# chongminggao/CIRS-codes

Measured on AMD Instinct MI355X. Metric: simulator env-steps/s (collect + PPO update in the timed region), KuaishouEnv, higher is better.
Workload: dtype f32 (policy/tracker; rollout on the fp32 MFMA, PPO head products fp32-accurate from two fp16 pieces per operand (3 f16 MFMAs per product), fp32 accumulate) + f64 (env rewards, GAE)

## Files before the change

### cirs-codes_amd/csrc/small_gemm.h

```cpp
#pragma once
#include "common.h"

namespace cirs {

typedef float sg_f32x16 __attribute__((ext_vector_type(16)));

template <bool kNT>
__device__ __forceinline__ void rows_gemm_body(int bx, int by, const float* __restrict__ X, int ldx, const float* __restrict__ W, int ldw,
                                               const float* __restrict__ bias, int R, int Kd, int N, int relu,
                                               const float* __restrict__ relu_of, int accumulate, float* __restrict__ Y, int ldy,
                                               const long* __restrict__ out_row) {
    const int lane = threadIdx.x, hi = lane >> 5, lo = lane & 31;
    const int row0 = bx * 32, n0 = by * 32;
    const int row = row0 + lo, n = n0 + lo;
    const bool row_ok = row < R, n_ok = n < N;
    sg_f32x16 acc;
    const float b = (bias && n_ok) ? bias[n] : 0.f;
#pragma unroll
    for (int s = 0; s < 16; ++s) acc[s] = b;
    const float* xr = X + (size_t)(row_ok ? row : 0) * ldx;
    if (kNT && (Kd & 31) == 0 && (ldx & 3) == 0 && ((uintptr_t)X & 15) == 0 && (ldw & 3) == 0 && ((uintptr_t)W & 15) == 0) {
        const float* wr = W + (size_t)(n_ok ? n : 0) * ldw;
        for (int kk = 0; kk < Kd; kk += 32) {
            float a[16], bv[16];
#pragma unroll
            for (int q = 0; q < 4; ++q) {
                const float4 t = *reinterpret_cast<const float4*>(xr + kk + 16 * hi + 4 * q);
                a[4 * q] = t.x; a[4 * q + 1] = t.y; a[4 * q + 2] = t.z; a[4 * q + 3] = t.w;
            }
#pragma unroll
            for (int q = 0; q < 4; ++q) {
                const float4 t = *reinterpret_cast<const float4*>(wr + kk + 16 * hi + 4 * q);
                bv[4 * q] = t.x; bv[4 * q + 1] = t.y; bv[4 * q + 2] = t.z; bv[4 * q + 3] = t.w;
            }
#pragma unroll
            for (int j = 0; j < 16; ++j)
                acc = __builtin_amdgcn_mfma_f32_32x32x2f32(row_ok ? a[j] : 0.f, n_ok ? bv[j] : 0.f, acc, 0, 0, 0);
        }
    } else if (!kNT && (Kd & 31) == 0 && (ldx & 3) == 0 && ((uintptr_t)X & 15) == 0) {
        for (int kk = 0; kk < Kd; kk += 32) {
            float a[16], bv[16];
#pragma unroll
            for (int q = 0; q < 4; ++q) {
                const float4 t = *reinterpret_cast<const float4*>(xr + kk + 16 * hi + 4 * q);
                a[4 * q] = t.x; a[4 * q + 1] = t.y; a[4 * q + 2] = t.z; a[4 * q + 3] = t.w;
            }
#pragma unroll
            for (int j = 0; j < 16; ++j) bv[j] = n_ok ? W[(size_t)(kk + 16 * hi + j) * ldw + n] : 0.f;
#pragma unroll
            for (int j = 0; j < 16; ++j) acc = __builtin_amdgcn_mfma_f32_32x32x2f32(row_ok ? a[j] : 0.f, bv[j], acc, 0, 0, 0);
        }
    } else {
        for (int kk = 0; kk < Kd; kk += 16) {
            float a[8], bv[8];
#pragma unroll
            for (int j = 0; j < 8; ++j) {
                const int kd = kk + 2 * j + hi;
                const bool k_ok = kd < Kd;
                a[j] = (row_ok && k_ok) ? xr[kd] : 0.f;
                bv[j] = 0.f;
                if (n_ok && k_ok) bv[j] = kNT ? W[(size_t)n * ldw + kd] : W[(size_t)kd * ldw + n];
            }
#pragma unroll
            for (int j = 0; j < 8; ++j) acc = __builtin_amdgcn_mfma_f32_32x32x2f32(a[j], bv[j], acc, 0, 0, 0);
        }
    }
    if (!n_ok) return;
#pragma unroll
    for (int s = 0; s < 16; ++s) {
        const int r = row0 + (s & 3) + 8 * (s >> 2) + 4 * hi;
        if (r >= R) continue;
        const size_t o = (size_t)(out_row ? out_row[r] : (long)r) * ldy + n;
        float v = acc[s];
        if (relu) v = fmaxf(v, 0.f);
        if (relu_of && !(relu_of[o] > 0.f)) v = 0.f;
        Y[o] = accumulate ? Y[o] + v : v;
    }
}

template <bool kNT>
static __global__ __launch_bounds__(64) void rows_gemm_kernel(const float* __restrict__ X, int ldx, const float* __restrict__ W, int ldw,
                                                              const float* __restrict__ bias, int R, int Kd, int N, int relu,
                                                              const float* __restrict__ relu_of, int accumulate,
                                                              float* __restrict__ Y, int ldy,
                                                              const long* __restrict__ out_row = nullptr) {
    rows_gemm_body<kNT>(blockIdx.x, blockIdx.y, X, ldx, W, ldw, bias, R, Kd, N, relu, relu_of, accumulate, Y, ldy, out_row);
}

static inline void launch_rows_gemm(bool nt, const float* X, int ldx, const float* W, int ldw, const float* bias, int R, int Kd, int N,
                                    int relu, const float* relu_of, int accumulate, float* Y, int ldy, hipStream_t s,
                                    const long* out_row = nullptr) {
    const dim3 grid(cdiv(R, 32), cdiv(N, 32));
    if (nt) hipLaunchKernelGGL(rows_gemm_kernel<true>, grid, dim3(64), 0, s, X, ldx, W, ldw, bias, R, Kd, N, relu, relu_of, accumulate, Y, ldy, out_row);
    else hipLaunchKernelGGL(rows_gemm_kernel<false>, grid, dim3(64), 0, s, X, ldx, W, ldw, bias, R, Kd, N, relu, relu_of, accumulate, Y, ldy, out_row);
}

constexpr int kDwMaxSlabs = 256;
__host__ inline int dwg_slabs(long R) {
    const long want = (R + 63) / 64;
    return (int)(want < 1 ? 1 : (want > kDwMaxSlabs ? kDwMaxSlabs : want));
}
__host__ inline size_t dwg_partial_floats(long R, int O, int K) { return (size_t)dwg_slabs(R) * O * (K + 1); }

__device__ __forceinline__ void dw_gemm_body(int bx, int slab, const float* __restrict__ dY, int ldy, const float* __restrict__ X, int ldx, int R,
                                             int O, int K, int rows_per_slab, float* __restrict__ partial) {
    const int lane = threadIdx.x, hi = lane >> 5, lo = lane & 31;
    const int k_tiles = (K + 31) / 32;
    const int o0 = (bx / k_tiles) * 32, k0 = (bx % k_tiles) * 32;
    const int r_beg = slab * rows_per_slab, r_end = min(R, r_beg + rows_per_slab);
    const int o = o0 + lo, k = k0 + lo;
    const bool o_ok = o < O, k_ok = k < K;
    sg_f32x16 acc;
#pragma unroll
    for (int s = 0; s < 16; ++s) acc[s] = 0.f;
    float bsum = 0.f;
    for (int r = r_beg; r < r_end; r += 64) {
        float a[32], b[32];
#pragma unroll
        for (int j = 0; j < 32; ++j) {
            const int rr = r + 2 * j + hi;
            const bool r_ok = rr < r_end;
            a[j] = (r_ok && o_ok) ? dY[(size_t)rr * ldy + o] : 0.f;
            b[j] = (r_ok && k_ok) ? X[(size_t)rr * ldx + k] : 0.f;
        }
#pragma unroll
        for (int j = 0; j < 32; ++j) {
            bsum += a[j];
            acc = __builtin_amdgcn_mfma_f32_32x32x2f32(a[j], b[j], acc, 0, 0, 0);
        }
    }
    float* out = partial + (size_t)slab * O * (K + 1);
    if (k_ok) {
#pragma unroll
        for (int s = 0; s < 16; ++s) {
            const int oo = o0 + (s & 3) + 8 * (s >> 2) + 4 * hi;
            if (oo < O) out[(size_t)oo * (K + 1) + k] = acc[s];
        }
    }
    if (k0 == 0) {
        bsum += __shfl_xor(bsum, 32, CIRS_WAVE);
        if (hi == 0 && o_ok) out[(size_t)o * (K + 1) + K] = bsum;
    }
}

static __global__ __launch_bounds__(64) void dw_gemm_kernel(const float* __restrict__ dY, int ldy, const float* __restrict__ X, int ldx, int R,
                                                            int O, int K, int rows_per_slab, float* __restrict__ partial) {
    dw_gemm_body(blockIdx.x, blockIdx.y, dY, ldy, X, ldx, R, O, K, rows_per_slab, partial);
}

struct RowsGemmArgs { const float* X; int ldx; const float* W; int ldw; const float* bias; int R, Kd, N, relu; const float* relu_of; int accumulate; float* Y; int ldy; };
struct DwGemmArgs { const float* dY; int ldy; const float* X; int ldx; int R, O, K, rows_per_slab; float* partial; };
template <bool kNT>
static __global__ __launch_bounds__(64) void rows_gemm_dw_kernel(RowsGemmArgs ra, int rgx, int rgy, DwGemmArgs da, int dgx) {
    const int b = blockIdx.x;
    if (b < rgx * rgy) {
        rows_gemm_body<kNT>(b % rgx, b / rgx, ra.X, ra.ldx, ra.W, ra.ldw, ra.bias, ra.R, ra.Kd, ra.N, ra.relu, ra.relu_of, ra.accumulate, ra.Y, ra.ldy,
                            nullptr);
    } else {
        const int q = b - rgx * rgy;
        dw_gemm_body(q % dgx, q / dgx, da.dY, da.ldy, da.X, da.ldx, da.R, da.O, da.K, da.rows_per_slab, da.partial);
    }
}

static __global__ __launch_bounds__(256) void dw_gemm_final(const float* __restrict__ partial, int n_slabs, int O, int K,
                                                            float* __restrict__ dW, float* __restrict__ db) {
    const int i = blockIdx.x * blockDim.x + threadIdx.x;
    const int n_out = O * (K + 1);
    if (i >= n_out) return;
    float acc = 0.f;
    for (int c0 = 0; c0 < n_slabs; c0 += 16) {
        float t16[16];
#pragma unroll
        for (int q = 0; q < 16; ++q) t16[q] = (c0 + q < n_slabs) ? partial[(size_t)(c0 + q) * n_out + i] : 0.f;
#pragma unroll
        for (int q = 0; q < 16; ++q) acc += t16[q];
    }
    const int o = i / (K + 1), k = i % (K + 1);
    if (k < K) dW[(size_t)o * K + k] = acc;
    else if (db) db[o] = acc;
}

static inline void launch_dw_gemm(const float* dY, int ldy, const float* X, int ldx, int R, int O, int K, float* dW, float* db,
                                  float* partial, hipStream_t s) {
    const int slabs = dwg_slabs(R);
    int rows_per_slab = (R + slabs - 1) / slabs;
    rows_per_slab = (rows_per_slab + 15) & ~15;
    const int tiles = cdiv(O, 32) * cdiv(K, 32);
    hipLaunchKernelGGL(dw_gemm_kernel, dim3(tiles, slabs), dim3(64), 0, s, dY, ldy, X, ldx, R, O, K, rows_per_slab, partial);
    hipLaunchKernelGGL(dw_gemm_final, dim3(cdiv(O * (K + 1), 256)), dim3(256), 0, s, partial, slabs, O, K, dW, db);
}


struct DwJob {
    const float* dY; int ldy; const float* X; int ldx; int O; int K;
    float* dW; float* db; int tile_begin; int part_off;
};
constexpr int kMaxDwJobs = 4;
struct DwJobs { DwJob j[kMaxDwJobs]; int n; int total_tiles; int total_out; };

__device__ __forceinline__ float dw_multi_fetch(int n_out, int part_off, int n_slabs, const float* __restrict__ partial, int i) {
    float acc = 0.f;
    for (int c0 = 0; c0 < n_slabs; c0 += 32) {
        float t32[32];
#pragma unroll
        for (int q = 0; q < 32; ++q) t32[q] = (c0 + q < n_slabs) ? partial[part_off + (size_t)(c0 + q) * n_out + i] : 0.f;
#pragma unroll
        for (int q = 0; q < 32; ++q) acc += t32[q];
    }
    return acc;
}
__device__ __forceinline__ float dw_multi_fetch(const DwJob& jb, int n_slabs, const float* __restrict__ partial, int i) {
    return dw_multi_fetch(jb.O * (jb.K + 1), jb.part_off, n_slabs, partial, i);
}

static __global__ __launch_bounds__(256) void dw_multi_final(DwJobs jobs, int n_slabs, const float* __restrict__ partial) {
    int i = blockIdx.x * blockDim.x + threadIdx.x;
    if (i >= jobs.total_out) return;
    int ji = 0;
    for (; ji < jobs.n; ++ji) {
        const int n_out = jobs.j[ji].O * (jobs.j[ji].K + 1);
        if (i < n_out) break;
        i -= n_out;
    }
    const DwJob jb = jobs.j[ji];
    const int n_out = jb.O * (jb.K + 1);
    const float acc = dw_multi_fetch(jb, n_slabs, partial, i);
    const int o = i / (jb.K + 1), k = i % (jb.K + 1);
    if (k < jb.K) jb.dW[(size_t)o * jb.K + k] = acc;
    else if (jb.db) jb.db[o] = acc;
}

constexpr int kMaxDwList = 3 + 6 * CIRS_MAX_TRACKER_LAYERS;
struct DwListJob { int O, K, part_off, diag; float* dW; float* db; };
struct DwList { DwListJob j[kMaxDwList]; int n, total_out, part_floats; };

static inline void launch_rows_gemm_dw(DwList& list, const float* dwX, int dw_ldx, int dwO, int dwK, float* dW, float* db, float* partial,
                                       bool nt, const float* X, int ldx, const float* W, int ldw, const float* bias, int R, int Kd, int N,
                                       int relu, const float* relu_of, int accumulate, float* Y, int ldy, hipStream_t s) {
    const int slabs = dwg_slabs(R);
    int rows_per_slab = (R + slabs - 1) / slabs;
    rows_per_slab = (rows_per_slab + 15) & ~15;
    DwListJob& jb = list.j[list.n++];
    jb.O = dwO; jb.K = dwK; jb.part_off = list.part_floats; jb.diag = 0; jb.dW = dW; jb.db = db;
    list.part_floats += slabs * dwO * (dwK + 1);
    list.total_out += dwO * (dwK + 1);
    const int tiles = cdiv(dwO, 32) * cdiv(dwK, 32);
    const RowsGemmArgs ra{X, ldx, W, ldw, bias, R, Kd, N, relu, relu_of, accumulate, Y, ldy};
    const DwGemmArgs da{X, ldx, dwX, dw_ldx, R, dwO, dwK, rows_per_slab, partial + jb.part_off};
    const int rgx = cdiv(R, 32), rgy = cdiv(N, 32);
    if (nt) hipLaunchKernelGGL(rows_gemm_dw_kernel<true>, dim3(rgx * rgy + tiles * slabs), dim3(64), 0, s, ra, rgx, rgy, da, tiles);
    else hipLaunchKernelGGL(rows_gemm_dw_kernel<false>, dim3(rgx * rgy + tiles * slabs), dim3(64), 0, s, ra, rgx, rgy, da, tiles);
}

static __global__ __launch_bounds__(256) void dw_list_final(DwList list, int n_slabs, const float* __restrict__ partial) {
    const int g = (blockIdx.x * blockDim.x + threadIdx.x) >> 3, q = threadIdx.x & 7;
    int i = g;
    const bool live = i < list.total_out;
    if (!live) i = 0;
    int O = 1, K = 0, part_off = 0, diag = 0;
    float* dW = nullptr;
    float* db = nullptr;
    bool found = false;
#pragma unroll
    for (int ji = 0; ji < kMaxDwList; ++ji) {
        if (ji < list.n && !found) {
            const int n_out_j = list.j[ji].O * (list.j[ji].K + 1);
            if (i < n_out_j) {
                O = list.j[ji].O; K = list.j[ji].K; part_off = list.j[ji].part_off; diag = list.j[ji].diag; dW = list.j[ji].dW; db = list.j[ji].db;
                found = true;
            } else {
                i -= n_out_j;
            }
        }
    }
    const int n_out = O * (K + 1);
    const int per = (n_slabs + 7) >> 3;
    const int c_beg = q * per, c_end = min(n_slabs, c_beg + per);
    float acc = 0.f;
    for (int c0 = c_beg; c0 < c_end; c0 += 16) {
        float t16[16];
#pragma unroll
        for (int u = 0; u < 16; ++u) t16[u] = (c0 + u < c_end) ? partial[part_off + (size_t)(c0 + u) * n_out + i] : 0.f;
#pragma unroll
        for (int u = 0; u < 16; ++u) acc += t16[u];
    }
    float tot = __shfl(acc, (threadIdx.x & 63) & 56, CIRS_WAVE);
#pragma unroll
    for (int u = 1; u < 8; ++u) tot += __shfl(acc, ((threadIdx.x & 63) & 56) | u, CIRS_WAVE);
    if (!live || q != 0) return;
    const int o = i / (K + 1), k = i % (K + 1);
    if (k < K) {
        if (!diag) dW[(size_t)o * K + k] = tot;
        else if (o == k) dW[o] = tot;
    } else if (db) {
        db[o] = tot;
    }
}

static inline void launch_dw_list_final(const DwList& list, int R, const float* partial, hipStream_t s) {
    hipLaunchKernelGGL(dw_list_final, dim3(cdiv(list.total_out * 8, 256)), dim3(256), 0, s, list, dwg_slabs(R), partial);
}

__host__ inline size_t dw_list_floats(long R, int O, int K) { return (size_t)dwg_slabs(R) * O * (K + 1); }

}
```

### cirs-codes_amd/csrc/tracker_bwd.hip

```cpp
#include <algorithm>
#include "tracker_rows.h"
#include "rng.h"

namespace cirs {

#ifdef CIRS_TBWD_PROF
__device__ unsigned long long g_tbwd_prof[64];
#define CIRS_BSTAMP(K) do { if ((int)blockIdx.x == 300 && threadIdx.x == 0) g_tbwd_prof[K] = __builtin_amdgcn_s_memtime(); } while (0)
__device__ unsigned long long g_tbwd_wg[2048 * 3];
#define CIRS_BWG(SEL, WHICH) do { if ((SEL) && threadIdx.x == 0 && blockIdx.x < 2048) { g_tbwd_wg[blockIdx.x * 3 + (WHICH)] = __builtin_amdgcn_s_memtime(); \
    if ((WHICH) == 0) { unsigned hw; asm volatile("s_getreg_b32 %0, hwreg(HW_REG_HW_ID)" : "=s"(hw)); unsigned xcc; asm volatile("s_getreg_b32 %0, hwreg(HW_REG_XCC_ID)" : "=s"(xcc)); g_tbwd_wg[blockIdx.x * 3 + 2] = ((unsigned long long)xcc << 32) | hw; } } } while (0)
#else
#define CIRS_BSTAMP(K) do { } while (0)
#define CIRS_BWG(SEL, WHICH) do { } while (0)
#endif
constexpr int kChunkRows = 256;

struct DropCfg {
    int on;
    uint32_t thr;
    float inv;
    uint64_t seed;
    int env_base;
};
__device__ __forceinline__ float drop_apply(const DropCfg& dc, float v, int env, int pos, int layer, int site, int elem) {
    return dropout_keep(dc.seed, (uint32_t)(dc.env_base + env), (uint32_t)pos, (uint32_t)layer, (uint32_t)site, (uint32_t)elem, dc.thr) ? v * dc.inv : 0.f;
}
template <int NH>
__global__ __launch_bounds__(256) void attn_fwd(const float* __restrict__ QKV, const int32_t* __restrict__ row_env,
                                                const int32_t* __restrict__ row_t, const int32_t* __restrict__ offsets, int R,
                                                int Lp, float* __restrict__ P, float* __restrict__ ATT, DropCfg dc, int layer,
                                                float* __restrict__ PM) {
    extern __shared__ __attribute__((aligned(16))) float smem[];
    constexpr int HD = tD / NH;
    const int lane = threadIdx.x & 63;
    const int r = blockIdx.x * 4 + (threadIdx.x >> 6);
    if (r >= R) return;
    float* ps = smem + (size_t)(threadIdx.x >> 6) * NH * Lp;
    const int p = row_t[r], base = offsets[row_env[r]];
    const float scale = 1.0f / sqrtf((float)HD);
    float q[tD];
    {
        const f32x4* q4 = reinterpret_cast<const f32x4*>(QKV + (size_t)r * 96);
#pragma unroll
        for (int d4 = 0; d4 < tD / 4; ++d4) {
            const f32x4 t = q4[d4];
            q[4 * d4] = t.x * scale; q[4 * d4 + 1] = t.y * scale; q[4 * d4 + 2] = t.z * scale; q[4 * d4 + 3] = t.w * scale;
        }
    }
    float mx[NH], sm[NH];
#pragma unroll
    for (int h = 0; h < NH; ++h) mx[h] = -INFINITY;
    float* Pr = P + (size_t)r * NH * Lp;
    for (int jp = lane; jp <= p; jp += CIRS_WAVE) {
        float k[tD];
        {
            const f32x4* k4 = reinterpret_cast<const f32x4*>(QKV + (size_t)(base + jp) * 96 + tD);
#pragma unroll
            for (int d4 = 0; d4 < tD / 4; ++d4) {
                const f32x4 t = k4[d4];
                k[4 * d4] = t.x; k[4 * d4 + 1] = t.y; k[4 * d4 + 2] = t.z; k[4 * d4 + 3] = t.w;
            }
        }
#pragma unroll
        for (int h = 0; h < NH; ++h) {
            float sc = 0.f;
#pragma unroll
            for (int d = 0; d < HD; ++d) sc = __builtin_fmaf(q[h * HD + d], k[h * HD + d], sc);
            ps[h * Lp + jp] = sc;
            mx[h] = fmaxf(mx[h], sc);
        }
    }
#pragma unroll
    for (int h = 0; h < NH; ++h) { mx[h] = wave_max_f32(mx[h]); sm[h] = 0.f; }
    for (int jp = lane; jp <= p; jp += CIRS_WAVE) {
#pragma unroll
        for (int h = 0; h < NH; ++h) {
            const float e = expf(ps[h * Lp + jp] - mx[h]);
            ps[h * Lp + jp] = e;
            sm[h] += e;
        }
    }
#pragma unroll
    for (int h = 0; h < NH; ++h) sm[h] = 1.0f / wave_sum_f32(sm[h]);
    for (int jp = lane; jp <= p; jp += CIRS_WAVE) {
#pragma unroll
        for (int h = 0; h < NH; ++h) {
            const float pr = ps[h * Lp + jp] * sm[h];
            Pr[h * Lp + jp] = pr;
            if (dc.on) {
                const float pm = drop_apply(dc, pr, row_env[r], p, layer, CIRS_DROP_ATTN, jp * NH + h);
                PM[(size_t)r * NH * Lp + h * Lp + jp] = pm;
                ps[h * Lp + jp] = pm;
            } else {
                ps[h * Lp + jp] = pr;
            }
        }
    }
    __builtin_amdgcn_wave_barrier();
    const int half = lane >> 5, d = lane & 31, h = d / HD;
    float acc = 0.f;
    for (int j0 = half; j0 <= p; j0 += 16) {
        float v8[8];
#pragma unroll
        for (int u = 0; u < 8; ++u) v8[u] = j0 + 2 * u <= p ? QKV[(size_t)(base + j0 + 2 * u) * 96 + 2 * tD + d] : 0.f;
#pragma unroll
        for (int u = 0; u < 8; ++u)
            if (j0 + 2 * u <= p) acc = __builtin_fmaf(ps[h * Lp + j0 + 2 * u], v8[u], acc);
    }
    acc += __shfl_xor(acc, 32, CIRS_WAVE);
    if (lane < tD) ATT[(size_t)r * tD + d] = acc;
}

template <int NH>
__global__ __launch_bounds__(256) void attn_bwd_q(const float* __restrict__ QKV, const float* __restrict__ P, const float* __restrict__ dATT,
                                                  const int32_t* __restrict__ row_env, const int32_t* __restrict__ row_t,
                                                  const int32_t* __restrict__ offsets, int R, int Lp, float* __restrict__ dS,
                                                  float* __restrict__ dQKV, const float* __restrict__ PM, float drop_inv) {
    constexpr int HD = tD / NH;
    const int lane = threadIdx.x & 63;
    const int r = blockIdx.x * 4 + (threadIdx.x >> 6);
    if (r >= R) return;
    const int p = row_t[r], base = offsets[row_env[r]];
    const float scale = 1.0f / sqrtf((float)HD);
    float da[tD];
    {
        const f32x4* a4 = reinterpret_cast<const f32x4*>(dATT + (size_t)r * tD);
#pragma unroll
        for (int d4 = 0; d4 < tD / 4; ++d4) {
            const f32x4 t = a4[d4];
            da[4 * d4] = t.x; da[4 * d4 + 1] = t.y; da[4 * d4 + 2] = t.z; da[4 * d4 + 3] = t.w;
        }
    }
    const float* Pr = P + (size_t)r * NH * Lp;
    float* dSr = dS + (size_t)r * NH * Lp;
    float dot[NH];
#pragma unroll
    for (int h = 0; h < NH; ++h) dot[h] = 0.f;
    for (int jp = lane; jp <= p; jp += CIRS_WAVE) {
        float v[tD];
        {
            const f32x4* v4 = reinterpret_cast<const f32x4*>(QKV + (size_t)(base + jp) * 96 + 2 * tD);
#pragma unroll
            for (int d4 = 0; d4 < tD / 4; ++d4) {
                const f32x4 t = v4[d4];
                v[4 * d4] = t.x; v[4 * d4 + 1] = t.y; v[4 * d4 + 2] = t.z; v[4 * d4 + 3] = t.w;
            }
        }
#pragma unroll
        for (int h = 0; h < NH; ++h) {
            float dp = 0.f;
#pragma unroll
            for (int d = 0; d < HD; ++d) dp = __builtin_fmaf(da[h * HD + d], v[h * HD + d], dp);
            if (PM) dp = PM[(size_t)r * NH * Lp + h * Lp + jp] != 0.f ? dp * drop_inv : 0.f;
            dSr[h * Lp + jp] = dp;
            dot[h] = __builtin_fmaf(Pr[h * Lp + jp], dp, dot[h]);
        }
    }
#pragma unroll
    for (int h = 0; h < NH; ++h) dot[h] = wave_sum_f32(dot[h]);
    extern __shared__ float smem_q[];
    float* sds = smem_q + (size_t)(threadIdx.x >> 6) * NH * Lp;
    for (int jp = lane; jp <= p; jp += CIRS_WAVE) {
#pragma unroll
        for (int h = 0; h < NH; ++h) {
            const float ds = Pr[h * Lp + jp] * (dSr[h * Lp + jp] - dot[h]);
            dSr[h * Lp + jp] = ds;
            sds[h * Lp + jp] = ds;
        }
    }
    __builtin_amdgcn_fence(__ATOMIC_RELEASE, "wavefront");
    __builtin_amdgcn_wave_barrier();
    __builtin_amdgcn_fence(__ATOMIC_ACQUIRE, "wavefront");
    const int half = lane >> 5, d = lane & (tD - 1), hd = d / HD;
    float acc = 0.f;
    for (int j0 = half; j0 <= p; j0 += 16) {
        float k8[8];
#pragma unroll
        for (int u = 0; u < 8; ++u) k8[u] = j0 + 2 * u <= p ? QKV[(size_t)(base + j0 + 2 * u) * 96 + tD + d] : 0.f;
#pragma unroll
        for (int u = 0; u < 8; ++u)
            if (j0 + 2 * u <= p) acc = __builtin_fmaf(sds[hd * Lp + j0 + 2 * u], k8[u], acc);
    }
    acc += __shfl_xor(acc, 32, CIRS_WAVE);
    if (lane < tD) dQKV[(size_t)r * 96 + d] = acc * scale;
}

template <int NH>
__global__ __launch_bounds__(256) void attn_bwd_kv(const float* __restrict__ QKV, const float* __restrict__ P, const float* __restrict__ dS,
                                                   const float* __restrict__ dATT, const int32_t* __restrict__ row_env,
                                                   const int32_t* __restrict__ row_t, const int32_t* __restrict__ offsets,
                                                   const int32_t* __restrict__ lens, int R, int Lp, float* __restrict__ dQKV) {
    constexpr int HD = tD / NH;
    const int lane = threadIdx.x & 63;
    const int r = blockIdx.x * 4 + (threadIdx.x >> 6);
    if (r >= R) return;
    const int b = row_env[r], pk = row_t[r], base = offsets[b], len = lens[b];
    const float scale = 1.0f / sqrtf((float)HD);
    const int d = lane & (tD - 1), which = lane >> 5, h = d / HD;
    const float* coef = (which == 0 ? dS : P) + ((size_t)base * NH + h) * Lp + pk;
    const float* vec = which == 0 ? QKV + (size_t)base * 96 + d : dATT + (size_t)base * tD + d;
    const size_t cstride = (size_t)NH * Lp, vstride = which == 0 ? 96 : tD;
    const float cs = which == 0 ? scale : 1.0f;
    float acc = 0.f;
    int p = pk;
    for (; p < len; p += 8) {
        float c8[8], v8[8];
#pragma unroll
        for (int u = 0; u < 8; ++u) {
            const bool ok = p + u < len;
            c8[u] = ok ? coef[(size_t)(p + u) * cstride] : 0.f;
            v8[u] = ok ? vec[(size_t)(p + u) * vstride] : 0.f;
        }
#pragma unroll
        for (int u = 0; u < 8; ++u)
            if (p + u < len) acc = __builtin_fmaf(c8[u] * cs, v8[u], acc);
    }
    dQKV[(size_t)r * 96 + tD + lane] = acc;
}

template <int NH> struct EpGeo {
    static constexpr int NW = NH < 4 ? NH : 4;
    static constexpr int SL = 64 / NW;
    static constexpr int HPL = NH / NW;
    static constexpr int HD = tD / NH;
    static constexpr int DPL = HPL * HD;
    __host__ __device__ static constexpr int strip(int Lp) { return (HPL * Lp) | 1; }
    __host__ __device__ static constexpr size_t keep_words(int Lp) { return 2 * (size_t)NH * Lp; }
    __host__ __device__ static constexpr size_t fwd_floats(int Lp) { return (size_t)Lp * 64 + (size_t)NW * (Lp + 1) * strip(Lp) + keep_words(Lp); }
    __host__ __device__ static constexpr size_t bwd_floats(int Lp) { return (size_t)Lp * 128 + (size_t)NW * (Lp + 1) * strip(Lp) + 2 * (size_t)NH * Lp + keep_words(Lp); }
};

__device__ __forceinline__ void ep_stage(float* __restrict__ dst, const float* __restrict__ src, int rows, int src_stride, int cols, int tid, int nt) {
    const int c4n = cols >> 2;
    for (int i = tid; i < rows * c4n; i += nt) {
        const int row = i / c4n, c4 = i - row * c4n;
        *reinterpret_cast<f32x4*>(dst + (size_t)row * cols + 4 * c4) = *reinterpret_cast<const f32x4*>(src + (size_t)row * src_stride + 4 * c4);
    }
}
template <int COLS, int NQ>
__device__ __forceinline__ void ep_stage_issue(f32x4 (&r)[NQ], const float* __restrict__ src, int rows, int src_stride, int tid) {
    constexpr int c4n = COLS >> 2;
    static_assert(NQ * 64 >= 32 * c4n, "registers for 32 rows");
    const int n = rows * c4n;
#pragma unroll
    for (int q = 0; q < NQ; ++q) {
        const int i = min(tid + 64 * q, n - 1), row = i / c4n, c4 = i - row * c4n;
        r[q] = *reinterpret_cast<const f32x4*>(src + (size_t)row * src_stride + 4 * c4);
    }
}
template <int COLS, int NQ>
__device__ __forceinline__ void ep_stage_commit(float* __restrict__ dst, const f32x4 (&r)[NQ], int rows, int tid) {
    constexpr int c4n = COLS >> 2;
    const int n = rows * c4n;
#pragma unroll
    for (int q = 0; q < NQ; ++q) {
        const int i = tid + 64 * q, row = i / c4n, c4 = i - row * c4n;
        if (i < n) *reinterpret_cast<f32x4*>(dst + (size_t)row * COLS + 4 * c4) = r[q];
    }
}
__device__ __forceinline__ void ep_wave_sync() {
    asm volatile("s_waitcnt lgkmcnt(0)" ::: "memory");
    __builtin_amdgcn_wave_barrier();
}
template <int N> __device__ __forceinline__ void ep_load(float (&v)[N], const float* __restrict__ src) {
#pragma unroll
    for (int d4 = 0; d4 < N / 4; ++d4) {
        const f32x4 t = *reinterpret_cast<const f32x4*>(src + 4 * d4);
        v[4 * d4] = t.x; v[4 * d4 + 1] = t.y; v[4 * d4 + 2] = t.z; v[4 * d4 + 3] = t.w;
    }
}
template <int N> __device__ __forceinline__ void ep_store(float* __restrict__ dst, const float (&v)[N], float a) {
#pragma unroll
    for (int d4 = 0; d4 < N / 4; ++d4)
        *reinterpret_cast<f32x4*>(dst + 4 * d4) = f32x4{v[4 * d4] * a, v[4 * d4 + 1] * a, v[4 * d4 + 2] * a, v[4 * d4 + 3] * a};
}
__device__ __forceinline__ float ep_exp2(float x) { return __builtin_amdgcn_exp2f(x); }
template <int HD> __device__ __forceinline__ float ep_dot(const float* a, const float* b) {
    float s = 0.f;
#pragma unroll
    for (int d = 0; d < HD; ++d) s = __builtin_fmaf(a[d], b[d], s);
    return s;
}
template <int NH>
__device__ __forceinline__ void ep_keep_build(uint32_t* __restrict__ sK, int len, int b, int layer, const DropCfg& dc, int tid, int nt) {
    for (int i = tid; i < len * NH * 2; i += nt) sK[i] = 0u;
    ep_wave_sync();
    const int half = (len + 1) >> 1;
    const int bpr = (((len + 1) * NH + 3) >> 2) + 1;
    for (int i = tid; i < half * bpr; i += nt) {
        const int fr = i / bpr, g0 = i - fr * bpr;
        const int pA = fr, pB = len - 1 - fr;
        const int nA = ((pA + 1) * NH + 3) >> 2, nB = pB > pA ? ((pB + 1) * NH + 3) >> 2 : 0;
        const bool inA = g0 < nA;
        const int p = inA ? pA : pB, g = inA ? g0 : g0 - nA;
        if (g0 < nA + nB) {
            const u32x4 r = dropout_block(dc.seed, (uint32_t)(dc.env_base + b), (uint32_t)p, (uint32_t)layer, (uint32_t)CIRS_DROP_ATTN, (uint32_t)g);
#pragma unroll
            for (int wd = 0; wd < 4; ++wd) {
                const int elem = 4 * g + wd, j = elem / NH, h = elem - j * NH;
                if (j <= p && block_word(r, (uint32_t)wd) >= dc.thr) atomicOr(&sK[(p * NH + h) * 2 + (j >> 5)], 1u << (j & 31));
            }
        }
    }
    ep_wave_sync();
}
template <int NH>
__device__ __forceinline__ void ep_keep_build_row(uint32_t* __restrict__ sK, int p, int b, int layer, const DropCfg& dc, int tid, int nt) {
    for (int i = tid; i < NH * 2; i += nt) sK[i] = 0u;
    __syncthreads();
    for (int g = tid; 4 * g < (p + 1) * NH; g += nt) {
        const u32x4 r = dropout_block(dc.seed, (uint32_t)(dc.env_base + b), (uint32_t)p, (uint32_t)layer, (uint32_t)CIRS_DROP_ATTN, (uint32_t)g);
#pragma unroll
        for (int wd = 0; wd < 4; ++wd) {
            const int elem = 4 * g + wd, j = elem / NH, h = elem - j * NH;
            if (j <= p && block_word(r, (uint32_t)wd) >= dc.thr) atomicOr(&sK[h * 2 + (j >> 5)], 1u << (j & 31));
        }
    }
    __syncthreads();
}
__device__ __forceinline__ bool ep_keep_bit(const uint32_t (&m)[2], int j) { return ((j < 32 ? m[0] : m[1]) >> (j & 31)) & 1u; }

template <int NH, bool kDrop>
__global__ __launch_bounds__(64) void attn_fwd_ep(const float* __restrict__ QKV, const int32_t* __restrict__ offsets,
                                                  const int32_t* __restrict__ lens, int Lp, float* __restrict__ ATT, DropCfg dc, int layer,
                                                  uint32_t* __restrict__ keep_out ) {
    using G = EpGeo<NH>;
    constexpr int HPL = G::HPL, DPL = G::DPL, HD = G::HD, SL = G::SL;
    extern __shared__ __attribute__((aligned(16))) float smem[];
    const int b = blockIdx.x, len = lens[b];
    if (len <= 0) return;
    const int lane = threadIdx.x, hg = lane / SL, slot = lane - hg * SL;
    const int base = offsets[b], STR = G::strip(Lp);
    float* sKV = smem;
    float* sS = smem + (size_t)Lp * 64;
    uint32_t* sK = reinterpret_cast<uint32_t*>(sS + (size_t)G::NW * (Lp + 1) * STR);
    const int len32 = min(len, 32);
    f32x4 st_kv[8];
    ep_stage_issue<64, 8>(st_kv, QKV + (size_t)base * 96 + tD, len32, 96, lane);
    if (kDrop) {
        ep_keep_build<NH>(sK, len, b, layer, dc, lane, 64);
        if (keep_out)
            for (int i = lane; i < len * NH * 2; i += 64) keep_out[(size_t)base * NH * 2 + i] = sK[i];
    }
    ep_stage_commit<64, 8>(sKV, st_kv, len32, lane);
    if (len > 32) ep_stage(sKV + 32 * 64, QKV + (size_t)(base + 32) * 96 + tD, len - 32, 96, 64, lane, 64);
    __syncthreads();
    const float scale = 1.0f / sqrtf((float)HD), qs = scale * 1.4426950408889634f;
    for (int s0 = 0; 2 * s0 < len; s0 += SL) {
        const int pA = s0 + slot, pB = len - 1 - pA;
        const bool actA = pA <= pB, actB = pA < pB;
        const int rA = actA ? pA : 0, rB = actB ? pB : 0;
        const int jn = len - s0;
        float* myA = sS + ((size_t)hg * (Lp + 1) + (actA ? pA : Lp)) * STR;
        float* myB = sS + ((size_t)hg * (Lp + 1) + (actB ? pB : Lp)) * STR;
        float qA[DPL], qB[DPL];
        ep_load(qA, QKV + (size_t)(base + rA) * 96 + hg * DPL);
        ep_load(qB, QKV + (size_t)(base + rB) * 96 + hg * DPL);
#pragma unroll
        for (int d = 0; d < DPL; ++d) { qA[d] *= qs; qB[d] *= qs; }
        float mxA[HPL], mxB[HPL], smA[HPL], smB[HPL];
#pragma unroll
        for (int h = 0; h < HPL; ++h) { mxA[h] = mxB[h] = -INFINITY; smA[h] = smB[h] = 0.f; }
        float kq[DPL];
        ep_load(kq, sKV + hg * DPL);
#pragma unroll 4
        for (int j = 0; j < jn; ++j) {
            float k[DPL];
#pragma unroll
            for (int d = 0; d < DPL; ++d) k[d] = kq[d];
            ep_load(kq, sKV + (size_t)(j + 1 < jn ? j + 1 : j) * 64 + hg * DPL);
            const bool inA = actA && j <= pA, inB = actB && j <= pB;
#pragma unroll
            for (int h = 0; h < HPL; ++h) {
                const float sa = ep_dot<HD>(qA + h * HD, k + h * HD), sb = ep_dot<HD>(qB + h * HD, k + h * HD);
                myA[h * Lp + j] = sa; myB[h * Lp + j] = sb;
                mxA[h] = inA ? fmaxf(mxA[h], sa) : mxA[h];
                mxB[h] = inB ? fmaxf(mxB[h], sb) : mxB[h];
            }
        }
        float accA[DPL], accB[DPL];
#pragma unroll
        for (int d = 0; d < DPL; ++d) accA[d] = accB[d] = 0.f;
        uint32_t kmA[HPL][2], kmB[HPL][2];
        if (kDrop) {
#pragma unroll
            for (int h = 0; h < HPL; ++h) {
                kmA[h][0] = sK[(rA * NH + hg * HPL + h) * 2]; kmA[h][1] = sK[(rA * NH + hg * HPL + h) * 2 + 1];
                kmB[h][0] = sK[(rB * NH + hg * HPL + h) * 2]; kmB[h][1] = sK[(rB * NH + hg * HPL + h) * 2 + 1];
            }
        }
        float vq[DPL];
        ep_load(vq, sKV + 32 + hg * DPL);
#pragma unroll 4
        for (int j = 0; j < jn; ++j) {
            float v[DPL];
#pragma unroll
            for (int d = 0; d < DPL; ++d) v[d] = vq[d];
            ep_load(vq, sKV + (size_t)(j + 1 < jn ? j + 1 : j) * 64 + 32 + hg * DPL);
            const bool inA = actA && j <= pA, inB = actB && j <= pB;
#pragma unroll
            for (int h = 0; h < HPL; ++h) {
                float ea = ep_exp2(myA[h * Lp + j] - mxA[h]), eb = ep_exp2(myB[h * Lp + j] - mxB[h]);
                ea = inA ? ea : 0.f; eb = inB ? eb : 0.f;
                smA[h] += ea; smB[h] += eb;
                if (kDrop) {
                    if (!ep_keep_bit(kmA[h], j)) ea = 0.f;
                    if (!ep_keep_bit(kmB[h], j)) eb = 0.f;
                }
#pragma unroll
                for (int d = 0; d < HD; ++d) {
                    accA[h * HD + d] = __builtin_fmaf(ea, v[h * HD + d], accA[h * HD + d]);
                    accB[h * HD + d] = __builtin_fmaf(eb, v[h * HD + d], accB[h * HD + d]);
                }
            }
        }
#pragma unroll
        for (int h = 0; h < HPL; ++h) {
            const float ia = (kDrop ? dc.inv : 1.0f) / smA[h], ib = (kDrop ? dc.inv : 1.0f) / smB[h];
#pragma unroll
            for (int d = 0; d < HD; ++d) { accA[h * HD + d] *= ia; accB[h * HD + d] *= ib; }
        }
        if (actA) ep_store(ATT + (size_t)(base + pA) * tD + hg * DPL, accA, 1.0f);
        if (actB) ep_store(ATT + (size_t)(base + pB) * tD + hg * DPL, accB, 1.0f);
    }
}

template <int NH, bool kDrop>
__global__ __launch_bounds__(64) void attn_bwd_ep(const float* __restrict__ QKV, const float* __restrict__ dATT,
                                                  const int32_t* __restrict__ offsets, const int32_t* __restrict__ lens, int Lp,
                                                  float* __restrict__ dQKV, DropCfg dc, int layer,
                                                  const uint32_t* __restrict__ keep_in ) {
    using G = EpGeo<NH>;
    constexpr int HPL = G::HPL, DPL = G::DPL, HD = G::HD, SL = G::SL;
    extern __shared__ __attribute__((aligned(16))) float smem[];
    const int b = blockIdx.x, len = lens[b];
    if (len <= 0) return;
    const int lane = threadIdx.x, hg = lane / SL, slot = lane - hg * SL;
    const int base = offsets[b], STR = G::strip(Lp);
    float* sQKV = smem;
    float* sdA = smem + (size_t)Lp * 96;
    float* sS = sdA + (size_t)Lp * 32;
    float* sM = sS + (size_t)G::NW * (Lp + 1) * STR;
    float* sI = sM + (size_t)NH * Lp;
    uint32_t* sK = reinterpret_cast<uint32_t*>(sI + (size_t)NH * Lp);
    CIRS_BWG(layer == 1, 0);
    CIRS_BSTAMP(39);
    const int len32 = min(len, 32);
    f32x4 st_q[12], st_d[4];
    ep_stage_issue<96, 12>(st_q, QKV + (size_t)base * 96, len32, 96, lane);
    ep_stage_issue<tD, 4>(st_d, dATT + (size_t)base * tD, len32, tD, lane);
    CIRS_BSTAMP(38);
    if (kDrop) {
        if (keep_in) {
            for (int i = lane; i < len * NH * 2; i += 64) sK[i] = keep_in[(size_t)base * NH * 2 + i];
        } else {
            ep_keep_build<NH>(sK, len, b, layer, dc, lane, 64);
        }
    }
    ep_stage_commit<96, 12>(sQKV, st_q, len32, lane);
    ep_stage_commit<tD, 4>(sdA, st_d, len32, lane);
    if (len > 32) {
        ep_stage(sQKV + 32 * 96, QKV + (size_t)(base + 32) * 96, len - 32, 96, 96, lane, 64);
        ep_stage(sdA + 32 * tD, dATT + (size_t)(base + 32) * tD, len - 32, tD, tD, lane, 64);
    }
    __syncthreads();
    CIRS_BSTAMP(40);
    const float scale = 1.0f / sqrtf((float)HD), qs = scale * 1.4426950408889634f;
    const float dinv = kDrop ? dc.inv : 1.0f;
    for (int s0 = 0; 2 * s0 < len; s0 += SL) {
        const int pA = s0 + slot, pB = len - 1 - pA;
        const bool actA = pA <= pB, actB = pA < pB;
        const int rA = actA ? pA : 0, rB = actB ? pB : 0;
        const int jn = len - s0;
        float* myA = sS + ((size_t)hg * (Lp + 1) + (actA ? pA : Lp)) * STR;
        float* myB = sS + ((size_t)hg * (Lp + 1) + (actB ? pB : Lp)) * STR;
        float qA[DPL], qB[DPL], daA[DPL], daB[DPL];
        ep_load(qA, sQKV + (size_t)rA * 96 + hg * DPL);
        ep_load(qB, sQKV + (size_t)rB * 96 + hg * DPL);
        ep_load(daA, sdA + (size_t)rA * tD + hg * DPL);
        ep_load(daB, sdA + (size_t)rB * tD + hg * DPL);
#pragma unroll
        for (int d = 0; d < DPL; ++d) { qA[d] *= qs; qB[d] *= qs; }
        float mxA[HPL], mxB[HPL], smA[HPL], smB[HPL], dotA[HPL], dotB[HPL];
#pragma unroll
        for (int h = 0; h < HPL; ++h) { mxA[h] = mxB[h] = -INFINITY; smA[h] = smB[h] = 0.f; dotA[h] = dotB[h] = 0.f; }
        uint32_t kmA[HPL][2], kmB[HPL][2];
        if (kDrop) {
#pragma unroll
            for (int h = 0; h < HPL; ++h) {
                kmA[h][0] = sK[(rA * NH + hg * HPL + h) * 2]; kmA[h][1] = sK[(rA * NH + hg * HPL + h) * 2 + 1];
                kmB[h][0] = sK[(rB * NH + hg * HPL + h) * 2]; kmB[h][1] = sK[(rB * NH + hg * HPL + h) * 2 + 1];
            }
        }
        float kq[DPL], vq[DPL];
        ep_load(kq, sQKV + 32 + hg * DPL);
#pragma unroll 4
        for (int j = 0; j < jn; ++j) {
            float k[DPL];
#pragma unroll
            for (int d = 0; d < DPL; ++d) k[d] = kq[d];
            ep_load(kq, sQKV + (size_t)(j + 1 < jn ? j + 1 : j) * 96 + 32 + hg * DPL);
            const bool inA = actA && j <= pA, inB = actB && j <= pB;
#pragma unroll
            for (int h = 0; h < HPL; ++h) {
                const float sa = ep_dot<HD>(qA + h * HD, k + h * HD), sb = ep_dot<HD>(qB + h * HD, k + h * HD);
                myA[h * Lp + j] = sa; myB[h * Lp + j] = sb;
                mxA[h] = inA ? fmaxf(mxA[h], sa) : mxA[h];
                mxB[h] = inB ? fmaxf(mxB[h], sb) : mxB[h];
            }
        }
        CIRS_BSTAMP(45);
        ep_load(vq, sQKV + 64 + hg * DPL);
#pragma unroll 4
        for (int j = 0; j < jn; ++j) {
            float v[DPL];
#pragma unroll
            for (int d = 0; d < DPL; ++d) v[d] = vq[d];
            ep_load(vq, sQKV + (size_t)(j + 1 < jn ? j + 1 : j) * 96 + 64 + hg * DPL);
            const bool inA = actA && j <= pA, inB = actB && j <= pB;
#pragma unroll
            for (int h = 0; h < HPL; ++h) {
                float ea = ep_exp2(myA[h * Lp + j] - mxA[h]), eb = ep_exp2(myB[h * Lp + j] - mxB[h]);
                ea = inA ? ea : 0.f; eb = inB ? eb : 0.f;
                myA[h * Lp + j] = ea; myB[h * Lp + j] = eb;
                smA[h] += ea; smB[h] += eb;
                float dpa = ep_dot<HD>(daA + h * HD, v + h * HD), dpb = ep_dot<HD>(daB + h * HD, v + h * HD);
                if (kDrop) {
                    dpa = (inA && ep_keep_bit(kmA[h], j)) ? dpa * dinv : 0.f;
                    dpb = (inB && ep_keep_bit(kmB[h], j)) ? dpb * dinv : 0.f;
                }
                dotA[h] = __builtin_fmaf(ea, dpa, dotA[h]);
                dotB[h] = __builtin_fmaf(eb, dpb, dotB[h]);
            }
        }
        CIRS_BSTAMP(46);
        float invA[HPL], invB[HPL];
#pragma unroll
        for (int h = 0; h < HPL; ++h) {
            invA[h] = 1.0f / smA[h]; invB[h] = 1.0f / smB[h];
            dotA[h] *= invA[h]; dotB[h] *= invB[h];
            if (actA) { sM[((size_t)hg * Lp + pA) * HPL + h] = mxA[h]; sI[((size_t)hg * Lp + pA) * HPL + h] = invA[h]; }
            if (actB) { sM[((size_t)hg * Lp + pB) * HPL + h] = mxB[h]; sI[((size_t)hg * Lp + pB) * HPL + h] = invB[h]; }
        }
        float dqA[DPL], dqB[DPL];
#pragma unroll
        for (int d = 0; d < DPL; ++d) dqA[d] = dqB[d] = 0.f;
        ep_load(kq, sQKV + 32 + hg * DPL);
        ep_load(vq, sQKV + 64 + hg * DPL);
#pragma unroll 4
        for (int j = 0; j < jn; ++j) {
            float k[DPL], v[DPL];
#pragma unroll
            for (int d = 0; d < DPL; ++d) { k[d] = kq[d]; v[d] = vq[d]; }
            ep_load(kq, sQKV + (size_t)(j + 1 < jn ? j + 1 : j) * 96 + 32 + hg * DPL);
            ep_load(vq, sQKV + (size_t)(j + 1 < jn ? j + 1 : j) * 96 + 64 + hg * DPL);
            const bool inA = actA && j <= pA, inB = actB && j <= pB;
#pragma unroll
            for (int h = 0; h < HPL; ++h) {
                float dpa = ep_dot<HD>(daA + h * HD, v + h * HD), dpb = ep_dot<HD>(daB + h * HD, v + h * HD);
                if (kDrop) {
                    dpa = (inA && ep_keep_bit(kmA[h], j)) ? dpa * dinv : 0.f;
                    dpb = (inB && ep_keep_bit(kmB[h], j)) ? dpb * dinv : 0.f;
                }
                float dsa = myA[h * Lp + j] * invA[h] * (dpa - dotA[h]), dsb = myB[h * Lp + j] * invB[h] * (dpb - dotB[h]);
                dsa = inA ? dsa : 0.f; dsb = inB ? dsb : 0.f;
                myA[h * Lp + j] = dsa; myB[h * Lp + j] = dsb;
#pragma unroll
                for (int d = 0; d < HD; ++d) {
                    dqA[h * HD + d] = __builtin_fmaf(dsa, k[h * HD + d], dqA[h * HD + d]);
                    dqB[h * HD + d] = __builtin_fmaf(dsb, k[h * HD + d], dqB[h * HD + d]);
                }
            }
        }
        if (actA) ep_store(dQKV + (size_t)(base + pA) * 96 + hg * DPL, dqA, scale);
        if (actB) ep_store(dQKV + (size_t)(base + pB) * 96 + hg * DPL, dqB, scale);
    }
    __syncthreads();
    CIRS_BSTAMP(41);
    for (int s0 = 0; 2 * s0 < len; s0 += SL) {
        const int jA = s0 + slot, jB = len - 1 - jA;
        const bool actA = jA <= jB, actB = jA < jB;
        const int rA = actA ? jA : 0, rB = actB ? jB : 0;
        float kA[DPL], kB[DPL], dKA[DPL], dVA[DPL], dKB[DPL], dVB[DPL];
        ep_load(kA, sQKV + (size_t)rA * 96 + 32 + hg * DPL);
        ep_load(kB, sQKV + (size_t)rB * 96 + 32 + hg * DPL);
#pragma unroll
        for (int d = 0; d < DPL; ++d) { kA[d] *= qs; kB[d] *= qs; dKA[d] = dVA[d] = dKB[d] = dVB[d] = 0.f; }
        float qn[DPL], dn[DPL];
        ep_load(qn, sQKV + (size_t)s0 * 96 + hg * DPL);
        ep_load(dn, sdA + (size_t)s0 * tD + hg * DPL);
#pragma unroll 4
        for (int pq = s0; pq < len; ++pq) {
            float q[DPL], da[DPL];
#pragma unroll
            for (int d = 0; d < DPL; ++d) { q[d] = qn[d]; da[d] = dn[d]; }
            ep_load(qn, sQKV + (size_t)(pq + 1 < len ? pq + 1 : pq) * 96 + hg * DPL);
            ep_load(dn, sdA + (size_t)(pq + 1 < len ? pq + 1 : pq) * tD + hg * DPL);
            const size_t st = ((size_t)hg * Lp + pq), ss = ((size_t)hg * (Lp + 1) + pq) * STR;
            const bool inA = actA && pq >= jA, inB = actB && pq >= jB;
#pragma unroll
            for (int h = 0; h < HPL; ++h) {
                const float m = sM[st * HPL + h], iv = sI[st * HPL + h];
                float pa = ep_exp2(fminf(ep_dot<HD>(q + h * HD, kA + h * HD) - m, 0.f)) * iv;
                float pb = ep_exp2(fminf(ep_dot<HD>(q + h * HD, kB + h * HD) - m, 0.f)) * iv;
                pa = inA ? pa : 0.f; pb = inB ? pb : 0.f;
                if (kDrop) {
                    const uint32_t* kw = sK + (pq * NH + hg * HPL + h) * 2;
                    pa = (inA && ((kw[rA >> 5] >> (rA & 31)) & 1u)) ? pa * dinv : 0.f;
                    pb = (inB && ((kw[rB >> 5] >> (rB & 31)) & 1u)) ? pb * dinv : 0.f;
                }
                float dsa = sS[ss + h * Lp + rA], dsb = sS[ss + h * Lp + rB];
                dsa = inA ? dsa : 0.f; dsb = inB ? dsb : 0.f;
#pragma unroll
                for (int d = 0; d < HD; ++d) {
                    dKA[h * HD + d] = __builtin_fmaf(dsa, q[h * HD + d], dKA[h * HD + d]);
                    dVA[h * HD + d] = __builtin_fmaf(pa, da[h * HD + d], dVA[h * HD + d]);
                    dKB[h * HD + d] = __builtin_fmaf(dsb, q[h * HD + d], dKB[h * HD + d]);
                    dVB[h * HD + d] = __builtin_fmaf(pb, da[h * HD + d], dVB[h * HD + d]);
                }
            }
        }
        if (actA) {
            float* o = dQKV + (size_t)(base + jA) * 96 + 32 + hg * DPL;
            ep_store(o, dKA, scale); ep_store(o + 32, dVA, 1.0f);
        }
        if (actB) {
            float* o = dQKV + (size_t)(base + jB) * 96 + 32 + hg * DPL;
            ep_store(o, dKB, scale); ep_store(o + 32, dVB, 1.0f);
        }
    }
    CIRS_BSTAMP(42);
    CIRS_BWG(layer == 1, 1);
}
#undef EP_KEEP

constexpr int kRowT = 132;
__device__ __forceinline__ void mm_block(sg_f32x16& acc, const float (&a)[16], const float* __restrict__ wr) {
    float bv[16];
    ep_load(bv, wr);
#pragma unroll
    for (int j = 0; j < 16; ++j) acc = __builtin_amdgcn_mfma_f32_32x32x2f32(a[j], bv[j], acc, 0, 0, 0);
}
__device__ __forceinline__ void acc_to_lds(float* __restrict__ sT, const sg_f32x16& acc, int col, int hi) {
#pragma unroll
    for (int s = 0; s < 16; ++s) sT[acc_row(s, hi) * kRowT + col] = acc[s];
}
__device__ __forceinline__ void ln_half_row(const float (&y)[16], const float* __restrict__ g, const float* __restrict__ b, int hi,
                                            float (&xh)[16], float (&out)[16], float& rs) {
    float sum = 0.f;
#pragma unroll
    for (int j = 0; j < 16; ++j) sum += y[j];
    sum += __shfl_xor(sum, 32, CIRS_WAVE);
    const float mean = sum * (1.0f / tD);
    float q = 0.f;
#pragma unroll
    for (int j = 0; j < 16; ++j) { const float t = y[j] - mean; q = __builtin_fmaf(t, t, q); }
    q += __shfl_xor(q, 32, CIRS_WAVE);
    rs = 1.0f / sqrtf(q * (1.0f / tD) + 1e-5f);
    float gg[16], bb[16];
    ep_load(gg, g + 16 * hi);
    ep_load(bb, b + 16 * hi);
#pragma unroll
    for (int j = 0; j < 16; ++j) { xh[j] = (y[j] - mean) * rs; out[j] = xh[j] * gg[j] + bb[j]; }
}

struct LayerFwdArgs {
    const float *ATT, *H;
    cirs_tracker_layer y;
    const float *win_next, *bin_next;
    float *XH1, *RS1, *H1N, *FF1, *XH2, *RS2, *Hout, *QKVnext;
    const int32_t *row_env, *row_t;
    int R, layer;
};
__device__ __forceinline__ void mm_regs(sg_f32x16& acc, const float (&a)[16], const float (&bv)[16]) {
#pragma unroll
    for (int j = 0; j < 16; ++j) acc = __builtin_amdgcn_mfma_f32_32x32x2f32(a[j], bv[j], acc, 0, 0, 0);
}
__device__ __forceinline__ void ln_apply(const float (&y)[16], const float (&gg)[16], const float (&bb)[16], float (&xh)[16], float (&out)[16], float& rs) {
    float sum = 0.f;
#pragma unroll
    for (int j = 0; j < 16; ++j) sum += y[j];
    sum += __shfl_xor(sum, 32, CIRS_WAVE);
    const float mean = sum * (1.0f / tD);
    float q = 0.f;
#pragma unroll
    for (int j = 0; j < 16; ++j) { const float t = y[j] - mean; q = __builtin_fmaf(t, t, q); }
    q += __shfl_xor(q, 32, CIRS_WAVE);
    rs = 1.0f / sqrtf(q * (1.0f / tD) + 1e-5f);
#pragma unroll
    for (int j = 0; j < 16; ++j) { xh[j] = (y[j] - mean) * rs; out[j] = xh[j] * gg[j] + bb[j]; }
}
template <bool kDrop>
__global__ __launch_bounds__(64) void layer_rows_fwd(LayerFwdArgs a, DropCfg dc) {
    __shared__ __attribute__((aligned(16))) float sT[10 * 1024];
    CIRS_BSTAMP(0);
    const int lane = threadIdx.x, hi = lane >> 5, lo = lane & 31;
    const int row0 = blockIdx.x * 32, row = row0 + lo;
    const bool row_ok = row < a.R;
    const size_t rr = (size_t)(row_ok ? row : 0);
    const int env = kDrop ? a.row_env[rr] : 0, pos = kDrop ? a.row_t[rr] : 0;
    float x[16], hrow[16], wo[16], w1[4][16], g1[16], be1[16];
    ep_load(x, a.ATT + rr * tD + 16 * hi);
    ep_load(wo, a.y.out_proj_w + (size_t)lo * tD + 16 * hi);
    ep_load(hrow, a.H + rr * tD + 16 * hi);
    ep_load(g1, a.y.norm1_w + 16 * hi);
    ep_load(be1, a.y.norm1_b + 16 * hi);
#pragma unroll
    for (int nt = 0; nt < 4; ++nt) ep_load(w1[nt], a.y.lin1_w + (size_t)(nt * 32 + lo) * tD + 16 * hi);
    const float bo = a.y.out_proj_b[lo], bl2 = a.y.lin2_b[lo];
    float bl1[4];
#pragma unroll
    for (int nt = 0; nt < 4; ++nt) bl1[nt] = a.y.lin1_b[nt * 32 + lo];
    if (!row_ok) {
#pragma unroll
        for (int j = 0; j < 16; ++j) x[j] = 0.f;
    }
    sg_f32x16 acc;
#pragma unroll
    for (int s = 0; s < 16; ++s) acc[s] = bo;
    CIRS_BSTAMP(1);
    mm_regs(acc, x, wo);
    CIRS_BSTAMP(2);
    acc_to_lds(sT, acc, lo, hi);
    __syncthreads();
    float w2[4][16];
#pragma unroll
    for (int kb = 0; kb < 4; ++kb) ep_load(w2[kb], a.y.lin2_w + (size_t)lo * tH + kb * 32 + 16 * hi);
    float y[16], xh[16], h1n[16], rs;
    {
        float t[16];
        ep_load(t, sT + lo * kRowT + 16 * hi);
#pragma unroll
        for (int j = 0; j < 16; ++j) {
            float v = t[j];
            if (kDrop) v = drop_apply(dc, v, env, pos, a.layer, CIRS_DROP_RES1, 16 * hi + j);
            y[j] = row_ok ? hrow[j] + v : 0.f;
        }
    }
    CIRS_BSTAMP(3);
    ln_apply(y, g1, be1, xh, h1n, rs);
    CIRS_BSTAMP(4);
    if (row_ok) {
        ep_store(a.XH1 + rr * tD + 16 * hi, xh, 1.0f);
        ep_store(a.H1N + rr * tD + 16 * hi, h1n, 1.0f);
        if (hi == 0) a.RS1[rr] = rs;
    } else {
#pragma unroll
        for (int j = 0; j < 16; ++j) h1n[j] = 0.f;
    }
    __syncthreads();
    CIRS_BSTAMP(5);
#pragma unroll
    for (int nt = 0; nt < 4; ++nt) {
        const int n = nt * 32 + lo;
#pragma unroll
        for (int s = 0; s < 16; ++s) acc[s] = bl1[nt];
        mm_regs(acc, h1n, w1[nt]);
#pragma unroll
        for (int s = 0; s < 16; ++s) acc[s] = fmaxf(acc[s], 0.f);
        acc_to_lds(sT, acc, n, hi);
    }
    __syncthreads();
    CIRS_BSTAMP(6);
    float g2[16], be2[16], wn[3][16], bn[3];
    ep_load(g2, a.y.norm2_w + 16 * hi);
    ep_load(be2, a.y.norm2_b + 16 * hi);
    if (a.win_next) {
#pragma unroll
        for (int nt = 0; nt < 3; ++nt) {
            ep_load(wn[nt], a.win_next + (size_t)(nt * 32 + lo) * tD + 16 * hi);
            bn[nt] = a.bin_next[nt * 32 + lo];
        }
    }
#pragma unroll
    for (int s = 0; s < 16; ++s) acc[s] = bl2;
#pragma unroll
    for (int kb = 0; kb < 4; ++kb) {
        float f[16];
        ep_load(f, sT + lo * kRowT + kb * 32 + 16 * hi);
#pragma unroll
        for (int j = 0; j < 16; ++j) {
            if (kDrop) f[j] = drop_apply(dc, f[j], env, pos, a.layer, CIRS_DROP_FF, kb * 32 + 16 * hi + j);
            if (!row_ok) f[j] = 0.f;
        }
        if (row_ok) ep_store(a.FF1 + rr * tH + kb * 32 + 16 * hi, f, 1.0f);
        mm_regs(acc, f, w2[kb]);
    }
    CIRS_BSTAMP(7);
    __syncthreads();
    acc_to_lds(sT, acc, lo, hi);
    __syncthreads();
    float hn[16];
    {
        float t[16];
        ep_load(t, sT + lo * kRowT + 16 * hi);
#pragma unroll
        for (int j = 0; j < 16; ++j) {
            float v = t[j];
            if (kDrop) v = drop_apply(dc, v, env, pos, a.layer, CIRS_DROP_RES2, 16 * hi + j);
            y[j] = row_ok ? h1n[j] + v : 0.f;
        }
    }
    CIRS_BSTAMP(8);
    ln_apply(y, g2, be2, xh, hn, rs);
    CIRS_BSTAMP(9);
    if (row_ok) {
        ep_store(a.XH2 + rr * tD + 16 * hi, xh, 1.0f);
        ep_store(a.Hout + rr * tD + 16 * hi, hn, 1.0f);
        if (hi == 0) a.RS2[rr] = rs;
    } else {
#pragma unroll
        for (int j = 0; j < 16; ++j) hn[j] = 0.f;
    }
    CIRS_BSTAMP(10);
    if (a.win_next) {
#pragma unroll
        for (int nt = 0; nt < 3; ++nt) {
            const int n = nt * 32 + lo;
#pragma unroll
            for (int s = 0; s < 16; ++s) acc[s] = bn[nt];
            mm_regs(acc, hn, wn[nt]);
#pragma unroll
            for (int s = 0; s < 16; ++s) {
                const int r = row0 + acc_row(s, hi);
                if (r < a.R) a.QKVnext[(size_t)r * 96 + n] = acc[s];
            }
        }
    }
    CIRS_BSTAMP(11);
}

template <bool kDrop>
__global__ __launch_bounds__(64) void embed_inproj(const float* __restrict__ x_hist, const float* __restrict__ pe,
                                                   const int32_t* __restrict__ row_env, const int32_t* __restrict__ row_t, int R, int L,
                                                   const float* __restrict__ win, const float* __restrict__ bin, float* __restrict__ H0,
                                                   float* __restrict__ QKV, DropCfg dc) {
    const int lane = threadIdx.x, hi = lane >> 5, lo = lane & 31;
    const int row0 = blockIdx.x * 32, row = row0 + lo;
    const bool row_ok = row < R;
    const size_t rr = (size_t)(row_ok ? row : 0);
    const int b = row_env[rr], p = row_t[rr];
    float x[16], pp[16], h[16];
    ep_load(x, x_hist + ((size_t)b * L + p) * tD + 16 * hi);
    ep_load(pp, pe + (size_t)p * tD + 16 * hi);
#pragma unroll
    for (int j = 0; j < 16; ++j) {
        float v = x[j] * 5.656854249492381f + pp[j];
        if (kDrop) v = drop_apply(dc, v, b, p, 0, CIRS_DROP_POS, 16 * hi + j);
        h[j] = row_ok ? v : 0.f;
    }
    if (row_ok) ep_store(H0 + rr * tD + 16 * hi, h, 1.0f);
    sg_f32x16 acc;
#pragma unroll
    for (int nt = 0; nt < 3; ++nt) {
        const int n = nt * 32 + lo;
        const float bias = bin[n];
#pragma unroll
        for (int s = 0; s < 16; ++s) acc[s] = bias;
        mm_block(acc, h, win + (size_t)n * tD + 16 * hi);
#pragma unroll
        for (int s = 0; s < 16; ++s) {
            const int r = row0 + acc_row(s, hi);
            if (r < R) QKV[(size_t)r * 96 + n] = acc[s];
        }
    }
}

__device__ __forceinline__ void load_wcols(float (&bv)[16], const float* __restrict__ W, int ldw, int k0, int n) {
#pragma unroll
    for (int j = 0; j < 16; ++j) bv[j] = W[(size_t)(k0 + j) * ldw + n];
}
__device__ __forceinline__ void ln_bwd_half_row(const float (&dout)[16], const float (&xh)[16], const float (&gg)[16], float rs, float (&dy)[16]) {
    float s1 = 0.f, s2 = 0.f, dxh[16];
#pragma unroll
    for (int j = 0; j < 16; ++j) { dxh[j] = dout[j] * gg[j]; s1 += dxh[j]; s2 = __builtin_fmaf(dxh[j], xh[j], s2); }
    s1 += __shfl_xor(s1, 32, CIRS_WAVE);
    s2 += __shfl_xor(s2, 32, CIRS_WAVE);
    const float m1 = s1 * (1.0f / tD), m2 = s2 * (1.0f / tD);
#pragma unroll
    for (int j = 0; j < 16; ++j) dy[j] = rs * (dxh[j] - m1 - xh[j] * m2);
}
struct LayerBwdArgs {
    const float *dHin, *dY1p, *dQKVp, *winp;
    float* dHout;
    int only_pre;
    cirs_tracker_layer y;
    const float *XH2, *RS2, *FF1, *XH1, *RS1;
    float *dB2, *dFF1, *dH1N, *dY1, *dB1, *dATT;
    const int32_t *row_env, *row_t;
    int R, layer;
};
template <int LDW> __device__ __forceinline__ void load_wcols_c(float (&bv)[16], const float* __restrict__ W, int k0, int n) {
#pragma unroll
    for (int j = 0; j < 16; ++j) bv[j] = W[(k0 + j) * LDW + n];
}
template <bool kDrop>
__global__ __launch_bounds__(64) void layer_rows_bwd(LayerBwdArgs a, DropCfg dc) {
    __shared__ __attribute__((aligned(16))) float sT[10 * 1024];
    CIRS_BSTAMP(20);
    const int lane = threadIdx.x, hi = lane >> 5, lo = lane & 31;
    const int row0 = blockIdx.x * 32, row = row0 + lo;
    const bool row_ok = row < a.R;
    const size_t rr = (size_t)(row_ok ? row : 0);
    const int env = kDrop ? a.row_env[rr] : 0, pos = kDrop ? a.row_t[rr] : 0;
    const float dinv = kDrop ? dc.inv : 1.0f;
    sg_f32x16 acc;
    float dh[16];
    if (a.dQKVp) {
        float q[3][16], res[16], bv[3][16];
        ep_load(res, a.dY1p + rr * tD + 16 * hi);
#pragma unroll
        for (int kb = 0; kb < 3; ++kb) {
            ep_load(q[kb], a.dQKVp + rr * 96 + kb * 32 + 16 * hi);
            load_wcols_c<tD>(bv[kb], a.winp, kb * 32 + 16 * hi, lo);
        }
#pragma unroll
        for (int s = 0; s < 16; ++s) acc[s] = 0.f;
#pragma unroll
        for (int kb = 0; kb < 3; ++kb) {
            if (!row_ok) {
#pragma unroll
                for (int j = 0; j < 16; ++j) q[kb][j] = 0.f;
            }
            mm_regs(acc, q[kb], bv[kb]);
        }
        acc_to_lds(sT, acc, lo, hi);
        __syncthreads();
        float t[16];
        ep_load(t, sT + lo * kRowT + 16 * hi);
#pragma unroll
        for (int j = 0; j < 16; ++j) {
            dh[j] = row_ok ? res[j] + t[j] : 0.f;
            if (kDrop && a.only_pre) dh[j] = drop_apply(dc, dh[j], env, pos, 0, CIRS_DROP_POS, 16 * hi + j);
        }
        if (row_ok) ep_store(a.dHout + rr * tD + 16 * hi, dh, 1.0f);
        if (a.only_pre) return;
        __syncthreads();
    } else {
        ep_load(dh, a.dHin + rr * tD + 16 * hi);
        if (!row_ok) {
#pragma unroll
            for (int j = 0; j < 16; ++j) dh[j] = 0.f;
        }
    }
    CIRS_BSTAMP(21);
    float xh2[16], g2[16], xh1[16], g1[16], w2[4][16], ffr[4][16];
    ep_load(xh2, a.XH2 + rr * tD + 16 * hi);
    ep_load(g2, a.y.norm2_w + 16 * hi);
    const float rs2 = a.RS2[rr], rs1 = a.RS1[rr];
#pragma unroll
    for (int nt = 0; nt < 4; ++nt) load_wcols_c<tH>(w2[nt], a.y.lin2_w, 16 * hi, nt * 32 + lo);
#pragma unroll
    for (int kb = 0; kb < 4; ++kb) ep_load(ffr[kb], a.FF1 + rr * tH + kb * 32 + 16 * hi);
    ep_load(xh1, a.XH1 + rr * tD + 16 * hi);
    ep_load(g1, a.y.norm1_w + 16 * hi);
    float dy2[16], db2[16];
    ln_bwd_half_row(dh, xh2, g2, rs2, dy2);
#pragma unroll
    for (int j = 0; j < 16; ++j) {
        if (!row_ok) dy2[j] = 0.f;
        db2[j] = kDrop ? drop_apply(dc, dy2[j], env, pos, a.layer, CIRS_DROP_RES2, 16 * hi + j) : dy2[j];
    }
    if (row_ok) ep_store(a.dB2 + rr * tD + 16 * hi, db2, 1.0f);
    CIRS_BSTAMP(22);
#pragma unroll
    for (int nt = 0; nt < 4; ++nt) {
#pragma unroll
        for (int s = 0; s < 16; ++s) acc[s] = 0.f;
        mm_regs(acc, db2, w2[nt]);
        acc_to_lds(sT, acc, nt * 32 + lo, hi);
    }
    float w1[4][16], wo[16];
#pragma unroll
    for (int kb = 0; kb < 4; ++kb) load_wcols_c<tD>(w1[kb], a.y.lin1_w, kb * 32 + 16 * hi, lo);
    load_wcols_c<tD>(wo, a.y.out_proj_w, 16 * hi, lo);
    __syncthreads();
    CIRS_BSTAMP(23);
    float f[4][16];
#pragma unroll
    for (int kb = 0; kb < 4; ++kb) {
        ep_load(f[kb], sT + lo * kRowT + kb * 32 + 16 * hi);
#pragma unroll
        for (int j = 0; j < 16; ++j) f[kb][j] = (row_ok && ffr[kb][j] > 0.f) ? f[kb][j] * dinv : 0.f;
        if (row_ok) ep_store(a.dFF1 + rr * tH + kb * 32 + 16 * hi, f[kb], 1.0f);
    }
    CIRS_BSTAMP(24);
#pragma unroll
    for (int s = 0; s < 16; ++s) acc[s] = 0.f;
#pragma unroll
    for (int kb = 0; kb < 4; ++kb) mm_regs(acc, f[kb], w1[kb]);
    __syncthreads();
    acc_to_lds(sT, acc, lo, hi);
    __syncthreads();
    CIRS_BSTAMP(25);
    float dh1n[16];
    {
        float t[16];
        ep_load(t, sT + lo * kRowT + 16 * hi);
#pragma unroll
        for (int j = 0; j < 16; ++j) dh1n[j] = row_ok ? dy2[j] + t[j] : 0.f;
        if (row_ok) ep_store(a.dH1N + rr * tD + 16 * hi, dh1n, 1.0f);
    }
    CIRS_BSTAMP(26);
    float dy1[16], db1[16];
    ln_bwd_half_row(dh1n, xh1, g1, rs1, dy1);
#pragma unroll
    for (int j = 0; j < 16; ++j) {
        if (!row_ok) dy1[j] = 0.f;
        db1[j] = kDrop ? drop_apply(dc, dy1[j], env, pos, a.layer, CIRS_DROP_RES1, 16 * hi + j) : dy1[j];
    }
    if (row_ok) {
        ep_store(a.dY1 + rr * tD + 16 * hi, dy1, 1.0f);
        if (kDrop) ep_store(a.dB1 + rr * tD + 16 * hi, db1, 1.0f);
    }
    CIRS_BSTAMP(27);
#pragma unroll
    for (int s = 0; s < 16; ++s) acc[s] = 0.f;
    mm_regs(acc, db1, wo);
    __syncthreads();
    acc_to_lds(sT, acc, lo, hi);
    __syncthreads();
    {
        float t[16];
        ep_load(t, sT + lo * kRowT + 16 * hi);
        if (row_ok) ep_store(a.dATT + rr * tD + 16 * hi, t, 1.0f);
    }
    CIRS_BSTAMP(28);
}

struct BwdScratch {
    float *G, *H[CIRS_MAX_TRACKER_LAYERS + 1];
    float *QKV[CIRS_MAX_TRACKER_LAYERS], *P[CIRS_MAX_TRACKER_LAYERS], *ATT[CIRS_MAX_TRACKER_LAYERS];
    float *XH1[CIRS_MAX_TRACKER_LAYERS], *RS1[CIRS_MAX_TRACKER_LAYERS], *H1N[CIRS_MAX_TRACKER_LAYERS], *FF1[CIRS_MAX_TRACKER_LAYERS];
    float *XH2[CIRS_MAX_TRACKER_LAYERS], *RS2[CIRS_MAX_TRACKER_LAYERS];
    float *T0, *T1, *T2, *T3, *T4, *T5, *dQKV, *dFF1, *dS, *partial, *GIN;
    float* LC;
    float* PM[CIRS_MAX_TRACKER_LAYERS];
    void* sort;
};

constexpr int kLastFloats = tD + 16 + 2 + 2;

static size_t bwd_partial_floats(const cirs_tracker_cfg* cfg, long R) {
    size_t f = dw_list_floats(R, 32, tD) + dw_list_floats(R, tD, tD) + dw_list_floats(R, tD, tD + 1);
    f += (size_t)cfg->nlayers * (2 * dw_list_floats(R, tD, tD) + dw_list_floats(R, tD, tH) + dw_list_floats(R, tH, tD) +
                                 dw_list_floats(R, tD, tD) + dw_list_floats(R, 96, tD));
    return f;
}

static size_t bwd_floats(const cirs_tracker_cfg* cfg, long R) {
    const long nl = cfg->nlayers, Lp = cfg->max_len, NH = cfg->nhead;
    size_t f = 0;
    f += (size_t)R * 32;
    f += (size_t)(nl + 1) * R * tD;
    f += (size_t)nl * R * (96 + NH * Lp + tD + tD + 1 + tD + tH + tD + 1);
    f += 6 * (size_t)R * tD + (size_t)R * 96 + (size_t)R * tH + (size_t)R * NH * Lp + 64;
    if (cfg->dropout_p > 0.f) f += (size_t)nl * R * NH * Lp + 64;
    f += bwd_partial_floats(cfg, R) + 4096;
    f += (size_t)R * (tD + 1);
    f += (size_t)R * kLastFloats;
    f += emb_sort_bytes(R + cfg->n_env) / 4 + 64;
    return f + 64 * 32;
}

static BwdScratch carve_bwd(void* ws, const cirs_tracker_cfg* cfg, long R) {
    float* p = (float*)ws;
    auto take = [&](size_t n) { float* r = p; p += (n + 3) & ~(size_t)3; return r; };
    const long nl = cfg->nlayers, Lp = cfg->max_len, NH = cfg->nhead;
    BwdScratch s;
    s.G = take((size_t)R * 32);
    for (int l = 0; l <= nl; ++l) s.H[l] = take((size_t)R * tD);
    for (int l = 0; l < nl; ++l) {
        s.QKV[l] = take((size_t)R * 96); s.P[l] = take((size_t)R * NH * Lp); s.ATT[l] = take((size_t)R * tD);
        s.XH1[l] = take((size_t)R * tD); s.RS1[l] = take(R); s.H1N[l] = take((size_t)R * tD); s.FF1[l] = take((size_t)R * tH);
        s.XH2[l] = take((size_t)R * tD); s.RS2[l] = take(R);
    }
    s.T0 = take((size_t)R * tD); s.T1 = take((size_t)R * tD); s.T2 = take((size_t)R * tD); s.T3 = take((size_t)R * tD);
    s.T4 = take((size_t)R * tD); s.T5 = take((size_t)R * tD);
    for (int l = 0; l < nl; ++l) s.PM[l] = cfg->dropout_p > 0.f ? take((size_t)R * NH * Lp) : nullptr;
    s.dQKV = take((size_t)R * 96); s.dFF1 = take((size_t)R * tH); s.dS = take((size_t)R * NH * Lp);
    s.partial = take(bwd_partial_floats(cfg, R) + 4096);
    s.GIN = take((size_t)R * (tD + 1));
    s.LC = take((size_t)R * kLastFloats);
    s.sort = (void*)take(emb_sort_bytes(R + cfg->n_env) / 4 + 64);
    return s;
}

}

#ifdef CIRS_TBWD_PROF
extern "C" int cirs_debug_tbwd_wg(unsigned long long* out_host) {
    return hipMemcpyFromSymbol(out_host, HIP_SYMBOL(cirs::g_tbwd_wg), 2048 * 3 * sizeof(unsigned long long)) == hipSuccess ? 0 : -2;
}
extern "C" int cirs_debug_tbwd_prof(unsigned long long* out_host64) {
    return hipMemcpyFromSymbol(out_host64, HIP_SYMBOL(cirs::g_tbwd_prof), 64 * sizeof(unsigned long long)) == hipSuccess ? 0 : -2;
}
#endif

namespace cirs {
__global__ __launch_bounds__(256) void prefix_last_rows_kernel(const float* __restrict__ ATT, const float* __restrict__ H, const int32_t* __restrict__ row_env,
                                                               const int32_t* __restrict__ row_t, const int32_t* __restrict__ offsets,
                                                               const int32_t* __restrict__ lens, int B, float* __restrict__ ATTc, float* __restrict__ Hc,
                                                               int32_t* __restrict__ env_c, int32_t* __restrict__ t_c) {
    const int e = blockIdx.x * 8 + (threadIdx.x >> 5), c = threadIdx.x & 31;
    if (e >= B) return;
    const int n = lens[e];
    const long r = n > 0 ? (long)offsets[e] + n - 1 : -1;
    ATTc[(size_t)e * tD + c] = r >= 0 ? ATT[r * tD + c] : 0.f;
    Hc[(size_t)e * tD + c] = r >= 0 ? H[r * tD + c] : 0.f;
    if (c == 0) { env_c[e] = r >= 0 ? row_env[r] : e; t_c[e] = r >= 0 ? row_t[r] : 0; }
}
__global__ __launch_bounds__(256) void prefix_decoder_kernel(const float* __restrict__ H, const int32_t* __restrict__ lens, int B, int S,
                                                             const float* __restrict__ dec_w, const float* __restrict__ dec_b,
                                                             float* __restrict__ out, long out_stride) {
    const int e = blockIdx.x * 4 + (threadIdx.x >> 6), j = threadIdx.x & 63;
    if (e >= B || j >= S) return;
    if (lens[e] <= 0) return;
    const float* h = H + (size_t)e * tD;
    float acc = dec_b[j];
#pragma unroll
    for (int k = 0; k < tD; ++k) acc = __builtin_fmaf(h[k], dec_w[(size_t)j * tD + k], acc);
    out[(size_t)e * out_stride + j] = acc;
}

constexpr int kPQS = 104;
constexpr int kPAS = 36;
struct PrefixEnvArgs {
    const float *x_hist, *pe;
    const int32_t *row_env, *row_t, *offsets, *lens;
    cirs_tracker_layer layer[CIRS_MAX_TRACKER_LAYERS];
    const float *dec_w, *dec_b;
    float* state_out;
    long state_stride;
    int nl, L, S;
    TrunkFuse tf;
};
template <int NH> __host__ __device__ constexpr size_t prefix_env_scratch_floats() {
    return (size_t)EpGeo<NH>::NW * 33 * EpGeo<NH>::strip(32) > (size_t)32 * kRowT ? (size_t)EpGeo<NH>::NW * 33 * EpGeo<NH>::strip(32) : (size_t)32 * kRowT;
}
constexpr int kRowBitWords = 6;
template <int NH> __host__ __device__ constexpr size_t prefix_env_lds_floats() {
    return (size_t)32 * kPQS + (size_t)32 * kPAS + prefix_env_scratch_floats<NH>() + EpGeo<NH>::keep_words(32) + 32 * kRowBitWords;
}

#define EP_KEEP(POS, ELEM) dropout_keep(dc.seed, (uint32_t)(dc.env_base + b), (uint32_t)(POS), (uint32_t)layer, (uint32_t)CIRS_DROP_ATTN, (uint32_t)(ELEM), dc.thr)
template <int NH, bool kDrop>
__device__ __forceinline__ void prefix_attn_all(const float* __restrict__ sQ, float* __restrict__ sS, float* __restrict__ sA, uint32_t* __restrict__ sK, int len,
                                                int b, int layer, const DropCfg& dc, int lane) {
    using G = EpGeo<NH>;
    constexpr int HPL = G::HPL, DPL = G::DPL, HD = G::HD, SL = G::SL, Lp = 32;
    const int hg = lane / SL, slot = lane - hg * SL, STR = G::strip(Lp);
    if (kDrop) ep_keep_build<NH>(sK, len, b, layer, dc, lane, 64);
    const float scale = 1.0f / sqrtf((float)HD), qs = scale * 1.4426950408889634f;
    for (int s0 = 0; 2 * s0 < len; s0 += SL) {
        const int pA = s0 + slot, pB = len - 1 - pA;
        const bool actA = pA <= pB, actB = pA < pB;
        const int rA = actA ? pA : 0, rB = actB ? pB : 0;
        const int jn = len - s0;
        float* myA = sS + ((size_t)hg * (Lp + 1) + (actA ? pA : Lp)) * STR;
        float* myB = sS + ((size_t)hg * (Lp + 1) + (actB ? pB : Lp)) * STR;
        float qA[DPL], qB[DPL];
        ep_load(qA, sQ + rA * kPQS + hg * DPL);
        ep_load(qB, sQ + rB * kPQS + hg * DPL);
#pragma unroll
        for (int d = 0; d < DPL; ++d) { qA[d] *= qs; qB[d] *= qs; }
        float mxA[HPL], mxB[HPL], smA[HPL], smB[HPL];
#pragma unroll
        for (int h = 0; h < HPL; ++h) { mxA[h] = mxB[h] = -INFINITY; smA[h] = smB[h] = 0.f; }
        float kq[DPL];
        ep_load(kq, sQ + 32 + hg * DPL);
#pragma unroll 4
        for (int j = 0; j < jn; ++j) {
            float k[DPL];
#pragma unroll
            for (int d = 0; d < DPL; ++d) k[d] = kq[d];
            ep_load(kq, sQ + (j + 1 < jn ? j + 1 : j) * kPQS + 32 + hg * DPL);
            const bool inA = actA && j <= pA, inB = actB && j <= pB;
#pragma unroll
            for (int h = 0; h < HPL; ++h) {
                const float sa = ep_dot<HD>(qA + h * HD, k + h * HD), sb = ep_dot<HD>(qB + h * HD, k + h * HD);
                myA[h * Lp + j] = sa; myB[h * Lp + j] = sb;
                mxA[h] = inA ? fmaxf(mxA[h], sa) : mxA[h];
                mxB[h] = inB ? fmaxf(mxB[h], sb) : mxB[h];
            }
        }
        float accA[DPL], accB[DPL];
#pragma unroll
        for (int d = 0; d < DPL; ++d) accA[d] = accB[d] = 0.f;
        uint32_t kmA[HPL][2], kmB[HPL][2];
        if (kDrop) {
#pragma unroll
            for (int h = 0; h < HPL; ++h) {
                kmA[h][0] = sK[(rA * NH + hg * HPL + h) * 2]; kmA[h][1] = sK[(rA * NH + hg * HPL + h) * 2 + 1];
                kmB[h][0] = sK[(rB * NH + hg * HPL + h) * 2]; kmB[h][1] = sK[(rB * NH + hg * HPL + h) * 2 + 1];
            }
        }
        float vq[DPL];
        ep_load(vq, sQ + 64 + hg * DPL);
#pragma unroll 4
        for (int j = 0; j < jn; ++j) {
            float v[DPL];
#pragma unroll
            for (int d = 0; d < DPL; ++d) v[d] = vq[d];
            ep_load(vq, sQ + (j + 1 < jn ? j + 1 : j) * kPQS + 64 + hg * DPL);
            const bool inA = actA && j <= pA, inB = actB && j <= pB;
#pragma unroll
            for (int h = 0; h < HPL; ++h) {
                float ea = ep_exp2(myA[h * Lp + j] - mxA[h]), eb = ep_exp2(myB[h * Lp + j] - mxB[h]);
                ea = inA ? ea : 0.f; eb = inB ? eb : 0.f;
                smA[h] += ea; smB[h] += eb;
                if (kDrop) {
                    if (!ep_keep_bit(kmA[h], j)) ea = 0.f;
                    if (!ep_keep_bit(kmB[h], j)) eb = 0.f;
                }
#pragma unroll
                for (int d = 0; d < HD; ++d) {
                    accA[h * HD + d] = __builtin_fmaf(ea, v[h * HD + d], accA[h * HD + d]);
                    accB[h * HD + d] = __builtin_fmaf(eb, v[h * HD + d], accB[h * HD + d]);
                }
            }
        }
#pragma unroll
        for (int h = 0; h < HPL; ++h) {
            const float ia = (kDrop ? dc.inv : 1.0f) / smA[h], ib = (kDrop ? dc.inv : 1.0f) / smB[h];
#pragma unroll
            for (int d = 0; d < HD; ++d) { accA[h * HD + d] *= ia; accB[h * HD + d] *= ib; }
        }
        if (actA) ep_store(sA + pA * kPAS + hg * DPL, accA, 1.0f);
        if (actB) ep_store(sA + pB * kPAS + hg * DPL, accB, 1.0f);
    }
}
template <int NH, bool kDrop>
__device__ __forceinline__ void prefix_attn_last(const float* __restrict__ sQ, float* __restrict__ sS, float* __restrict__ sA, uint32_t* __restrict__ sK, int len,
                                                 int b, int layer, const DropCfg& dc, int lane) {
    constexpr int HD = tD / NH;
    const int p = len - 1;
    if (kDrop) ep_keep_build_row<NH>(sK, p, b, layer, dc, lane, 64);
    const float scale = 1.0f / sqrtf((float)HD), qs = scale * 1.4426950408889634f;
    {
        const int j = lane & 31;
        for (int h = lane >> 5; h < NH; h += 2) {
            float q[HD], k[HD];
            ep_load(q, sQ + p * kPQS + h * HD);
            ep_load(k, sQ + j * kPQS + 32 + h * HD);
#pragma unroll
            for (int d = 0; d < HD; ++d) q[d] *= qs;
            sS[h * 32 + j] = ep_dot<HD>(q, k);
        }
    }
    __syncthreads();
    if (lane < 32) {
        const int h = lane / HD;
        float sc[32];
        ep_load(sc, sS + h * 32);
        float mx = -INFINITY;
#pragma unroll
        for (int j = 0; j < 32; ++j) mx = j <= p ? fmaxf(mx, sc[j]) : mx;
        float sm = 0.f, acc = 0.f;
        const uint32_t km = kDrop ? sK[h * 2] : 0u;
#pragma unroll
        for (int j = 0; j < 32; ++j) {
            const bool in = j <= p;
            float e = ep_exp2(sc[j] - mx);
            e = in ? e : 0.f;
            sm += e;
            if (kDrop) {
                if (!((km >> j) & 1u)) e = 0.f;
            }
            acc = __builtin_fmaf(e, sQ[j * kPQS + 64 + lane], acc);
        }
        acc *= (kDrop ? dc.inv : 1.0f) / sm;
        sA[p * kPAS + lane] = acc;
    }
    __syncthreads();
}
#undef EP_KEEP
__device__ __forceinline__ void prefix_row_bits(uint32_t* __restrict__ sB, int r_begin, int n_rows, int env, int pos_of_lane, int layer, const DropCfg& dc, int lane) {
    for (int i = lane; i < 32 * kRowBitWords; i += 64) sB[i] = 0u;
    __syncthreads();
    for (int i0 = 0; i0 < n_rows * 48; i0 += 64) {
        const int i = i0 + lane, rl = i / 48, idx = i - rl * 48;
        const int pos = __shfl(pos_of_lane, (r_begin + rl) & 31, CIRS_WAVE);
        if (i < n_rows * 48) {
            const int site = idx < 8 ? (int)CIRS_DROP_RES1 : (idx < 40 ? (int)CIRS_DROP_FF : (int)CIRS_DROP_RES2);
            const int g = idx < 8 ? idx : (idx < 40 ? idx - 8 : idx - 40);
            const u32x4 r = dropout_block(dc.seed, (uint32_t)(dc.env_base + env), (uint32_t)pos, (uint32_t)layer, (uint32_t)site, (uint32_t)g);
            uint32_t m = 0u;
#pragma unroll
            for (int wd = 0; wd < 4; ++wd) m |= block_word(r, (uint32_t)wd) >= dc.thr ? 1u << wd : 0u;
            atomicOr(&sB[rl * kRowBitWords + (idx >> 3)], m << (4 * (idx & 7)));
        }
    }
    __syncthreads();
}
template <bool kDrop>
__device__ __forceinline__ void prefix_chain(const cirs_tracker_layer& y, const float* __restrict__ win_next, const float* __restrict__ bin_next, int layer,
                                             const DropCfg& dc, const uint32_t* __restrict__ myB, bool row_ok, int lo, int hi, const float* __restrict__ sA,
                                             float* __restrict__ sT, float* __restrict__ sQ, float (&hrow)[16]) {
    uint32_t kb1 = 0u, kbf[4] = {0u, 0u, 0u, 0u}, kb2 = 0u;
    if (kDrop) {
        kb1 = (myB[0] >> (16 * hi)) & 0xFFFFu;
#pragma unroll
        for (int kb = 0; kb < 4; ++kb) kbf[kb] = (myB[1 + kb] >> (16 * hi)) & 0xFFFFu;
        kb2 = (myB[5] >> (16 * hi)) & 0xFFFFu;
    }
    float x[16], wo[16], w1[4][16], g1[16], be1[16];
    ep_load(wo, y.out_proj_w + (size_t)lo * tD + 16 * hi);
    ep_load(g1, y.norm1_w + 16 * hi);
    ep_load(be1, y.norm1_b + 16 * hi);
#pragma unroll
    for (int nt = 0; nt < 4; ++nt) ep_load(w1[nt], y.lin1_w + (size_t)(nt * 32 + lo) * tD + 16 * hi);
    const float bo = y.out_proj_b[lo], bl2 = y.lin2_b[lo];
    float bl1[4];
#pragma unroll
    for (int nt = 0; nt < 4; ++nt) bl1[nt] = y.lin1_b[nt * 32 + lo];
    ep_load(x, sA + lo * kPAS + 16 * hi);
    if (!row_ok) {
#pragma unroll
        for (int j = 0; j < 16; ++j) x[j] = 0.f;
    }
    sg_f32x16 acc;
#pragma unroll
    for (int s = 0; s < 16; ++s) acc[s] = bo;
    mm_regs(acc, x, wo);
    acc_to_lds(sT, acc, lo, hi);
    __syncthreads();
    float w2[4][16];
#pragma unroll
    for (int kb = 0; kb < 4; ++kb) ep_load(w2[kb], y.lin2_w + (size_t)lo * tH + kb * 32 + 16 * hi);
    float yv[16], xh[16], h1n[16], rs;
    {
        float t[16];
        ep_load(t, sT + lo * kRowT + 16 * hi);
#pragma unroll
        for (int j = 0; j < 16; ++j) {
            float v = t[j];
            if (kDrop) v = ((kb1 >> j) & 1u) ? v * dc.inv : 0.f;
            yv[j] = row_ok ? hrow[j] + v : 0.f;
        }
    }
    ln_apply(yv, g1, be1, xh, h1n, rs);
    if (!row_ok) {
#pragma unroll
        for (int j = 0; j < 16; ++j) h1n[j] = 0.f;
    }
    __syncthreads();
#pragma unroll
    for (int nt = 0; nt < 4; ++nt) {
#pragma unroll
        for (int s = 0; s < 16; ++s) acc[s] = bl1[nt];
        mm_regs(acc, h1n, w1[nt]);
#pragma unroll
        for (int s = 0; s < 16; ++s) acc[s] = fmaxf(acc[s], 0.f);
        acc_to_lds(sT, acc, nt * 32 + lo, hi);
    }
    __syncthreads();
    float g2[16], be2[16], wn[3][16], bn[3];
    ep_load(g2, y.norm2_w + 16 * hi);
    ep_load(be2, y.norm2_b + 16 * hi);
    if (win_next) {
#pragma unroll
        for (int nt = 0; nt < 3; ++nt) {
            ep_load(wn[nt], win_next + (size_t)(nt * 32 + lo) * tD + 16 * hi);
            bn[nt] = bin_next[nt * 32 + lo];
        }
    }
#pragma unroll
    for (int s = 0; s < 16; ++s) acc[s] = bl2;
#pragma unroll
    for (int kb = 0; kb < 4; ++kb) {
        float f[16];
        ep_load(f, sT + lo * kRowT + kb * 32 + 16 * hi);
#pragma unroll
        for (int j = 0; j < 16; ++j) {
            if (kDrop) f[j] = ((kbf[kb] >> j) & 1u) ? f[j] * dc.inv : 0.f;
            if (!row_ok) f[j] = 0.f;
        }
        mm_regs(acc, f, w2[kb]);
    }
    __syncthreads();
    acc_to_lds(sT, acc, lo, hi);
    __syncthreads();
    {
        float t[16];
        ep_load(t, sT + lo * kRowT + 16 * hi);
#pragma unroll
        for (int j = 0; j < 16; ++j) {
            float v = t[j];
            if (kDrop) v = ((kb2 >> j) & 1u) ? v * dc.inv : 0.f;
            yv[j] = row_ok ? h1n[j] + v : 0.f;
        }
    }
    ln_apply(yv, g2, be2, xh, hrow, rs);
    if (!row_ok) {
#pragma unroll
        for (int j = 0; j < 16; ++j) hrow[j] = 0.f;
    }
    if (win_next) {
#pragma unroll
        for (int nt = 0; nt < 3; ++nt) {
#pragma unroll
            for (int s = 0; s < 16; ++s) acc[s] = bn[nt];
            mm_regs(acc, hrow, wn[nt]);
#pragma unroll
            for (int s = 0; s < 16; ++s) sQ[acc_row(s, hi) * kPQS + nt * 32 + lo] = acc[s];
        }
    }
    __syncthreads();
}
template <int NH, bool kDrop>
__global__ __launch_bounds__(64) void prefix_env_kernel(PrefixEnvArgs a, DropCfg dc) {
    extern __shared__ __attribute__((aligned(16))) float smem[];
    float* sQ = smem;
    float* sA = sQ + 32 * kPQS;
    float* sX = sA + 32 * kPAS;
    uint32_t* sK = reinterpret_cast<uint32_t*>(sX + prefix_env_scratch_floats<NH>());
    uint32_t* sB = sK + EpGeo<NH>::keep_words(32);
    const int e = blockIdx.x, len = a.lens[e];
    if (len <= 0) return;
    CIRS_BSTAMP(40);
    const int lane = threadIdx.x, hi = lane >> 5, lo = lane & 31;
    const int base = a.offsets[e];
    const bool row_ok = lo < len;
    const size_t rr = (size_t)base + (row_ok ? lo : 0);
    const int b = a.row_env[rr], p = a.row_t[rr];
    float h[16];
    {
        float x[16], pp[16];
        ep_load(x, a.x_hist + ((size_t)b * a.L + p) * tD + 16 * hi);
        ep_load(pp, a.pe + (size_t)p * tD + 16 * hi);
#pragma unroll
        for (int j = 0; j < 16; ++j) {
            float v = x[j] * 5.656854249492381f + pp[j];
            if (kDrop) v = drop_apply(dc, v, b, p, 0, CIRS_DROP_POS, 16 * hi + j);
            h[j] = row_ok ? v : 0.f;
        }
        sg_f32x16 acc;
        const float* win = a.layer[0].in_proj_w;
#pragma unroll
        for (int nt = 0; nt < 3; ++nt) {
            const int n = nt * 32 + lo;
            const float bias = a.layer[0].in_proj_b[n];
#pragma unroll
            for (int s = 0; s < 16; ++s) acc[s] = bias;
            mm_block(acc, h, win + (size_t)n * tD + 16 * hi);
#pragma unroll
            for (int s = 0; s < 16; ++s) sQ[acc_row(s, hi) * kPQS + n] = acc[s];
        }
    }
    __syncthreads();
    CIRS_BSTAMP(41);
    for (int l = 0; l < a.nl; ++l) {
        const bool last = l + 1 == a.nl;
        if (last) prefix_attn_last<NH, kDrop>(sQ, sX, sA, sK, len, e, l, dc, lane);
        else {
            prefix_attn_all<NH, kDrop>(sQ, sX, sA, sK, len, e, l, dc, lane);
            __syncthreads();
        }
        CIRS_BSTAMP(42 + 2 * l);
        if (kDrop) prefix_row_bits(sB, last ? len - 1 : 0, last ? 1 : len, b, p, l, dc, lane);
        prefix_chain<kDrop>(a.layer[l], last ? nullptr : a.layer[l + 1].in_proj_w, last ? nullptr : a.layer[l + 1].in_proj_b, l, dc,
                            sB + (last ? 0 : lo) * kRowBitWords, row_ok, lo, hi, sA, sX, sQ, h);
        CIRS_BSTAMP(43 + 2 * l);
    }
    if (lo == len - 1) ep_store(sA + 16 * hi, h, 1.0f);
    __syncthreads();
    float sval = 0.f;
    if (lane < a.S) {
        float acc = a.dec_b[lane];
#pragma unroll
        for (int k = 0; k < tD; ++k) acc = __builtin_fmaf(sA[k], a.dec_w[(size_t)lane * tD + k], acc);
        a.state_out[(size_t)e * a.state_stride + lane] = acc;
        sval = acc;
    }
    CIRS_BSTAMP(50);
    if (a.tf.on) {
        if (a.tf.skip && a.tf.skip[e]) {
            a.tf.h2[(size_t)e * kH + lane] = 0.f;
            if (lane == 0 && a.tf.value) a.tf.value[e] = 0.f;
            return;
        }
        float *xs = sX, *hs = sX + kH;
        if (lane < a.S) xs[lane] = sval;
        trunk_compute(a.tf.cfg, a.tf.w, xs, hs, lane, e, a.tf.h2, a.tf.value, nullptr);
    }
}

template <int NH>
__device__ __forceinline__ void last_keep_build(uint32_t* __restrict__ sK, const int32_t* __restrict__ lens, int e0, int E, int Lp, int layer,
                                                const DropCfg& dc, int tid) {
    constexpr int EPW = 64 / NH;
    for (int i = tid; i < EPW * NH * 2; i += 64) sK[i] = 0u;
    __syncthreads();
    const int gmax = (Lp * NH + 3) >> 2;
    for (int i = tid; i < EPW * gmax; i += 64) {
        const int el = i / gmax, g = i - el * gmax, e = e0 + el;
        const int len = e < E ? lens[e] : 0;
        if (4 * g < len * NH) {
            const int p = len - 1;
            const u32x4 r = dropout_block(dc.seed, (uint32_t)(dc.env_base + e), (uint32_t)p, (uint32_t)layer, (uint32_t)CIRS_DROP_ATTN, (uint32_t)g);
#pragma unroll
            for (int wd = 0; wd < 4; ++wd) {
                const int elem = 4 * g + wd, j = elem / NH, h = elem - j * NH;
                if (j <= p && block_word(r, (uint32_t)wd) >= dc.thr) atomicOr(&sK[(el * NH + h) * 2 + (j >> 5)], 1u << (j & 31));
            }
        }
    }
    __syncthreads();
}
template <int NH, bool kDrop>
__global__ __launch_bounds__(64) void attn_last_fwd(const float* __restrict__ QKV, const float* __restrict__ H, const int32_t* __restrict__ row_env,
                                                    const int32_t* __restrict__ row_t, const int32_t* __restrict__ offsets,
                                                    const int32_t* __restrict__ lens, int E, int Lp, float* __restrict__ ATTc, float* __restrict__ Hc,
                                                    float* __restrict__ stats, int32_t* __restrict__ env_c, int32_t* __restrict__ t_c, DropCfg dc, int layer) {
    constexpr int HD = tD / NH, EPW = 64 / NH;
    __shared__ uint32_t sK[EPW * NH * 2];
    const int tid = threadIdx.x, el = tid / NH, h = tid - el * NH, e0 = blockIdx.x * EPW, e = e0 + el;
    if (kDrop) last_keep_build<NH>(sK, lens, e0, E, Lp, layer, dc, tid);
    if (e >= E) return;
    const int len = lens[e];
    float acc[HD], hrow[HD];
    if (len <= 0) {
#pragma unroll
        for (int d = 0; d < HD; ++d) acc[d] = 0.f;
        ep_store(ATTc + (size_t)e * tD + h * HD, acc, 1.0f);
        ep_store(Hc + (size_t)e * tD + h * HD, acc, 1.0f);
        stats[((size_t)e * NH + h) * 2] = 0.f; stats[((size_t)e * NH + h) * 2 + 1] = 0.f;
        if (h == 0) { env_c[e] = e; t_c[e] = 0; }
        return;
    }
    const int p = len - 1;
    const size_t base = (size_t)offsets[e];
    const float* rows = QKV + base * 96 + h * HD;
    const float scale = 1.0f / sqrtf((float)HD), qs = scale * 1.4426950408889634f;
    float q[HD];
    ep_load(q, rows + (size_t)p * 96);
    ep_load(hrow, H + (base + p) * tD + h * HD);
#pragma unroll
    for (int d = 0; d < HD; ++d) q[d] *= qs;
    float mx = -INFINITY;
#pragma unroll 4
    for (int j = 0; j <= p; ++j) {
        float k[HD];
        ep_load(k, rows + (size_t)j * 96 + 32);
        mx = fmaxf(mx, ep_dot<HD>(q, k));
    }
    uint32_t km[2] = {0u, 0u};
    if (kDrop) { km[0] = sK[(el * NH + h) * 2]; km[1] = sK[(el * NH + h) * 2 + 1]; }
    float sm = 0.f;
#pragma unroll
    for (int d = 0; d < HD; ++d) acc[d] = 0.f;
#pragma unroll 4
    for (int j = 0; j <= p; ++j) {
        float k[HD], v[HD];
        ep_load(k, rows + (size_t)j * 96 + 32);
        ep_load(v, rows + (size_t)j * 96 + 64);
        float ex = ep_exp2(ep_dot<HD>(q, k) - mx);
        sm += ex;
        if (kDrop) {
            if (!ep_keep_bit(km, j)) ex = 0.f;
        }
#pragma unroll
        for (int d = 0; d < HD; ++d) acc[d] = __builtin_fmaf(ex, v[d], acc[d]);
    }
    const float ia = (kDrop ? dc.inv : 1.0f) / sm;
#pragma unroll
    for (int d = 0; d < HD; ++d) acc[d] *= ia;
    ep_store(ATTc + (size_t)e * tD + h * HD, acc, 1.0f);
    ep_store(Hc + (size_t)e * tD + h * HD, hrow, 1.0f);
    stats[((size_t)e * NH + h) * 2] = mx; stats[((size_t)e * NH + h) * 2 + 1] = 1.0f / sm;
    if (h == 0) { env_c[e] = row_env[base + p]; t_c[e] = row_t[base + p]; }
}
template <int NH, bool kDrop>
__global__ __launch_bounds__(64) void attn_last_bwd(const float* __restrict__ QKV, const float* __restrict__ dATTc, const float* __restrict__ dY1c,
                                                    const float* __restrict__ stats, const int32_t* __restrict__ offsets, const int32_t* __restrict__ lens,
                                                    int E, int Lp, float* __restrict__ dQKV, float* __restrict__ dY1, DropCfg dc, int layer) {
    constexpr int HD = tD / NH, EPW = 64 / NH;
    __shared__ uint32_t sK[EPW * NH * 2];
    const int tid = threadIdx.x, el = tid / NH, h = tid - el * NH, e0 = blockIdx.x * EPW, e = e0 + el;
    if (kDrop) last_keep_build<NH>(sK, lens, e0, E, Lp, layer, dc, tid);
    if (e >= E) return;
    const int len = lens[e];
    if (len <= 0) return;
    const int p = len - 1;
    const size_t base = (size_t)offsets[e];
    const float* rows = QKV + base * 96 + h * HD;
    const float scale = 1.0f / sqrtf((float)HD), qs = scale * 1.4426950408889634f, dinv = kDrop ? dc.inv : 1.0f;
    float qr[HD], q[HD], da[HD], res[HD], zero[HD];
    ep_load(qr, rows + (size_t)p * 96);
    ep_load(da, dATTc + (size_t)e * tD + h * HD);
    ep_load(res, dY1c + (size_t)e * tD + h * HD);
#pragma unroll
    for (int d = 0; d < HD; ++d) { q[d] = qr[d] * qs; zero[d] = 0.f; }
    const float mx = stats[((size_t)e * NH + h) * 2], inv = stats[((size_t)e * NH + h) * 2 + 1];
    uint32_t km[2] = {0u, 0u};
    if (kDrop) { km[0] = sK[(el * NH + h) * 2]; km[1] = sK[(el * NH + h) * 2 + 1]; }
    float dot = 0.f;
#pragma unroll 4
    for (int j = 0; j <= p; ++j) {
        float k[HD], v[HD];
        ep_load(k, rows + (size_t)j * 96 + 32);
        ep_load(v, rows + (size_t)j * 96 + 64);
        const float ex = ep_exp2(ep_dot<HD>(q, k) - mx);
        float dp = ep_dot<HD>(da, v);
        if (kDrop) dp = ep_keep_bit(km, j) ? dp * dinv : 0.f;
        dot = __builtin_fmaf(ex, dp, dot);
    }
    dot *= inv;
    float dq[HD];
#pragma unroll
    for (int d = 0; d < HD; ++d) dq[d] = 0.f;
    float* orow = dQKV + base * 96 + h * HD;
    float* yrow = dY1 + base * tD + h * HD;
#pragma unroll 2
    for (int j = 0; j <= p; ++j) {
        float k[HD], v[HD];
        ep_load(k, rows + (size_t)j * 96 + 32);
        ep_load(v, rows + (size_t)j * 96 + 64);
        const float pj = ep_exp2(ep_dot<HD>(q, k) - mx) * inv;
        float dp = ep_dot<HD>(da, v), pm = pj;
        if (kDrop) {
            const bool keep = ep_keep_bit(km, j);
            dp = keep ? dp * dinv : 0.f;
            pm = keep ? pj * dinv : 0.f;
        }
        const float ds = pj * (dp - dot);
#pragma unroll
        for (int d = 0; d < HD; ++d) dq[d] = __builtin_fmaf(ds, k[d], dq[d]);
        ep_store(orow + (size_t)j * 96 + 32, qr, ds * scale);
        ep_store(orow + (size_t)j * 96 + 64, da, pm);
        if (j < p) {
            ep_store(orow + (size_t)j * 96, zero, 1.0f);
            ep_store(yrow + (size_t)j * tD, zero, 1.0f);
        }
    }
    ep_store(orow + (size_t)p * 96, dq, scale);
    ep_store(yrow + (size_t)p * tD, res, 1.0f);
}
__global__ __launch_bounds__(256) void dstate_last_rows(const float* __restrict__ dstate_last, const int32_t* __restrict__ lens, int E, int S,
                                                        float* __restrict__ G) {
    const long i = blockIdx.x * (long)blockDim.x + threadIdx.x;
    if (i >= (long)E * S) return;
    G[i] = lens[i / S] > 0 ? dstate_last[i] : 0.f;
}
__global__ __launch_bounds__(256) void dstate_last_full(const float* __restrict__ dstate_last, const int32_t* __restrict__ row_env,
                                                        const int32_t* __restrict__ offsets, const int32_t* __restrict__ lens, int R, int S,
                                                        float* __restrict__ G) {
    const long i = blockIdx.x * (long)blockDim.x + threadIdx.x;
    if (i >= (long)R * S) return;
    const int r = (int)(i / S), s = (int)(i % S), b = row_env[r];
    G[i] = r == offsets[b] + lens[b] - 1 ? dstate_last[(size_t)b * S + s] : 0.f;
}
}

extern "C" int64_t cirs_tracker_backward_workspace_bytes(const cirs_tracker_cfg* cfg, int32_t n_rows) {
    if (!cfg || n_rows <= 0) return 0;
    return (int64_t)cirs::bwd_floats(cfg, n_rows) * 4;
}

static inline size_t spread_dyn_lds(long n_blocks, size_t static_bytes, size_t dyn_bytes) {
    if (n_blocks > cirs::device_cu_count()) return dyn_bytes;
    const size_t want = 81 * 1024;
    return static_bytes + dyn_bytes >= want ? dyn_bytes : want - static_bytes;
}
template <typename K> static inline void lds_optin(K k, size_t dyn) {
    if (dyn > 8 * 1024) (void)hipFuncSetAttribute(reinterpret_cast<const void*>(k), hipFuncAttributeMaxDynamicSharedMemorySize, (int)dyn);
}
#define CIRS_LAUNCH_SPREAD(KERNEL, GRID, STATIC_B, DYN_B, STREAM, ...)                                  \
    do {                                                                                               \
        const size_t dyn_ = spread_dyn_lds((long)(GRID), (STATIC_B), (DYN_B));                         \
        if (dyn_ != (size_t)(DYN_B)) lds_optin(KERNEL, dyn_);                                          \
        hipLaunchKernelGGL(KERNEL, dim3(GRID), dim3(64), dyn_, STREAM, __VA_ARGS__);                   \
    } while (0)

static int tracker_rows_impl(const cirs_tracker_cfg* cfg, const cirs_tracker_weights* w, const cirs_tracker_state* st,
                             const int32_t* users, const int64_t* act, const double* rew, const int32_t* row_env,
                             const int32_t* row_t, const int32_t* offsets, const int32_t* lens, int32_t n_rows,
                             const float* dstate, const cirs_tracker_grads* grads, void* workspace,
                             int64_t workspace_bytes, void* stream, float* state_out, int64_t state_stride, const float* dstate_last = nullptr,
                             const cirs::TrunkFuse* ptf = nullptr, int* ptf_fused = nullptr) {
    using namespace cirs;
    CIRS_REQUIRE(cfg && w && st && row_env && row_t && offsets && lens && workspace, "null argument");
    CIRS_REQUIRE(state_out || (users && act && rew && (dstate || dstate_last) && grads), "null argument");
    if (cfg->dim_model != tD || cfg->d_hid != tH) return fail(CIRS_E_UNSUPPORTED, "dim_model == 32 and d_hid == 128 only");
    CIRS_REQUIRE(cfg->nhead == 1 || cfg->nhead == 2 || cfg->nhead == 4 || cfg->nhead == 8, "nhead must be 1,2,4,8");
    CIRS_REQUIRE(n_rows > 0, "n_rows must be positive");
    const int n_carve = dstate_last && cfg->n_env > n_rows ? cfg->n_env : n_rows;
    CIRS_REQUIRE(workspace_bytes >= cirs_tracker_backward_workspace_bytes(cfg, n_carve), "workspace too small");
    hipStream_t s = (hipStream_t)stream;
    const int R = n_rows, B = cfg->n_env, S = cfg->dim_state, L = cfg->max_len, NH = cfg->nhead, nl = cfg->nlayers;
    BwdScratch sc = carve_bwd(workspace, cfg, n_carve);
    auto g1 = [&](long n) { return dim3(cdiv(n, 256)); };

    DwList dwl{};
#define ATT_DISPATCH_SH(KERNEL, SHMEM, ...)                                                               \
    do {                                                                                                  \
        switch (NH) {                                                                                     \
            case 1: hipLaunchKernelGGL(KERNEL<1>, dim3(cdiv(R, 4)), dim3(256), SHMEM, s, __VA_ARGS__); break; \
            case 2: hipLaunchKernelGGL(KERNEL<2>, dim3(cdiv(R, 4)), dim3(256), SHMEM, s, __VA_ARGS__); break; \
            case 4: hipLaunchKernelGGL(KERNEL<4>, dim3(cdiv(R, 4)), dim3(256), SHMEM, s, __VA_ARGS__); break; \
            default: hipLaunchKernelGGL(KERNEL<8>, dim3(cdiv(R, 4)), dim3(256), SHMEM, s, __VA_ARGS__); break; \
        }                                                                                                 \
    } while (0)
#define ATT_DISPATCH(KERNEL, ...) ATT_DISPATCH_SH(KERNEL, 0, __VA_ARGS__)
    auto ep_bytes = [&](bool bwd) -> size_t {
        switch (NH) {
            case 1: return 4 * (bwd ? EpGeo<1>::bwd_floats(L) : EpGeo<1>::fwd_floats(L));
            case 2: return 4 * (bwd ? EpGeo<2>::bwd_floats(L) : EpGeo<2>::fwd_floats(L));
            case 4: return 4 * (bwd ? EpGeo<4>::bwd_floats(L) : EpGeo<4>::fwd_floats(L));
            default: return 4 * (bwd ? EpGeo<8>::bwd_floats(L) : EpGeo<8>::fwd_floats(L));
        }
    };
    const bool ep = L <= 64 && ep_bytes(true) <= 64 * 1024 && !getenv("CIRS_TRACKER_ATTN_ROWS");
#define ATT_EP1(KERNEL, N, BWD, ...)                                                                                            \
    do {                                                                                                                        \
        if (dc.on) CIRS_LAUNCH_SPREAD((KERNEL<N, true>), B, 0, ep_bytes(BWD), s, __VA_ARGS__);       \
        else CIRS_LAUNCH_SPREAD((KERNEL<N, false>), B, 0, ep_bytes(BWD), s, __VA_ARGS__);           \
    } while (0)
#define ATT_EP(KERNEL, BWD, ...)                                  \
    do {                                                          \
        switch (NH) {                                             \
            case 1: ATT_EP1(KERNEL, 1, BWD, __VA_ARGS__); break;  \
            case 2: ATT_EP1(KERNEL, 2, BWD, __VA_ARGS__); break;  \
            case 4: ATT_EP1(KERNEL, 4, BWD, __VA_ARGS__); break;  \
            default: ATT_EP1(KERNEL, 8, BWD, __VA_ARGS__); break; \
        }                                                         \
    } while (0)

    DropCfg dc{};
    if (cfg->dropout_p > 0.f) {
        CIRS_REQUIRE(cfg->dropout_p < 1.f, "dropout_p must be in [0, 1)");
        dc.on = 1; dc.thr = dropout_threshold(cfg->dropout_p); dc.inv = 1.0f / (1.0f - cfg->dropout_p);
        dc.seed = cfg->dropout_seed; dc.env_base = cfg->drop_env_base;
    }
    if (state_out && ep && L <= 32 && S <= 64 && !getenv("CIRS_TRACKER_PREFIX_LAUNCHES")) {
        PrefixEnvArgs pa{};
        pa.x_hist = st->x_hist; pa.pe = w->pe; pa.row_env = row_env; pa.row_t = row_t; pa.offsets = offsets; pa.lens = lens;
        for (int l = 0; l < nl; ++l) pa.layer[l] = w->layer[l];
        pa.dec_w = w->dec_w; pa.dec_b = w->dec_b; pa.state_out = state_out; pa.state_stride = (long)state_stride; pa.nl = nl; pa.L = L; pa.S = S;
        if (ptf && ptf->on) {
            CIRS_REQUIRE(ptf->cfg.hidden == kH && ptf->cfg.dim_state == S && ptf->h2, "prefix states: trunk shape mismatch");
            pa.tf = *ptf;
            if (ptf_fused) *ptf_fused = 1;
        }
#define PREFIX_ENV(N)                                                                                                                        \
    do {                                                                                                                                     \
        const size_t sh = std::max<size_t>(4 * prefix_env_lds_floats<N>(), 40 * 1024);           \
        if (dc.on) hipLaunchKernelGGL((prefix_env_kernel<N, true>), dim3(B), dim3(64), sh, s, pa, dc);                                        \
        else hipLaunchKernelGGL((prefix_env_kernel<N, false>), dim3(B), dim3(64), sh, s, pa, dc);                                             \
    } while (0)
        switch (NH) {
            case 1: PREFIX_ENV(1); break;
            case 2: PREFIX_ENV(2); break;
            case 4: PREFIX_ENV(4); break;
            default: PREFIX_ENV(8); break;
        }
#undef PREFIX_ENV
        CIRS_CHECK_LAUNCH("prefix_env_kernel");
        return CIRS_OK;
    }
    if (dc.on) CIRS_LAUNCH_SPREAD(embed_inproj<true>, cdiv(R, 32), 0, 0, s, st->x_hist, w->pe, row_env, row_t, R, L, w->layer[0].in_proj_w,
                                  w->layer[0].in_proj_b, sc.H[0], sc.QKV[0], dc);
    else CIRS_LAUNCH_SPREAD(embed_inproj<false>, cdiv(R, 32), 0, 0, s, st->x_hist, w->pe, row_env, row_t, R, L, w->layer[0].in_proj_w,
                            w->layer[0].in_proj_b, sc.H[0], sc.QKV[0], dc);
    const bool top_last = dstate_last && ep && nl >= 2 && !getenv("CIRS_TRACKER_LAST_FULL");
    float *dY1c = sc.LC, *att_stats = sc.LC + (size_t)B * tD;
    int32_t *env_c = reinterpret_cast<int32_t*>(att_stats + (size_t)B * 16), *t_c = env_c + B;
#define ATT_LAST1(KERNEL, N, ...)                                                                                        \
    do {                                                                                                                 \
        if (dc.on) hipLaunchKernelGGL((KERNEL<N, true>), dim3(cdiv(B, 64 / N)), dim3(64), 0, s, __VA_ARGS__);             \
        else hipLaunchKernelGGL((KERNEL<N, false>), dim3(cdiv(B, 64 / N)), dim3(64), 0, s, __VA_ARGS__);                  \
    } while (0)
#define ATT_LAST(KERNEL, ...)                                  \
    do {                                                       \
        switch (NH) {                                          \
            case 1: ATT_LAST1(KERNEL, 1, __VA_ARGS__); break;  \
            case 2: ATT_LAST1(KERNEL, 2, __VA_ARGS__); break;  \
            case 4: ATT_LAST1(KERNEL, 4, __VA_ARGS__); break;  \
            default: ATT_LAST1(KERNEL, 8, __VA_ARGS__); break; \
        }                                                      \
    } while (0)
    for (int l = 0; l < nl; ++l) {
        const cirs_tracker_layer& y = w->layer[l];
        if (top_last && l == nl - 1) {
            float* Hc = sc.T1;
            ATT_LAST(attn_last_fwd, (const float*)sc.QKV[l], (const float*)sc.H[l], row_env, row_t, offsets, lens, B, L, sc.ATT[l], Hc, att_stats, env_c, t_c,
                     dc, l);
            LayerFwdArgs fa{sc.ATT[l], Hc, y, nullptr, nullptr, sc.XH1[l], sc.RS1[l], sc.H1N[l], sc.FF1[l], sc.XH2[l], sc.RS2[l], sc.H[l + 1], nullptr,
                            env_c, t_c, B, l};
            if (dc.on) CIRS_LAUNCH_SPREAD(layer_rows_fwd<true>, cdiv(B, 32), 40 * 1024, 0, s, fa, dc);
            else CIRS_LAUNCH_SPREAD(layer_rows_fwd<false>, cdiv(B, 32), 40 * 1024, 0, s, fa, dc);
            continue;
        }
        if (ep) ATT_EP(attn_fwd_ep, false, (const float*)sc.QKV[l], offsets, lens, L, sc.ATT[l], dc, l, (dc.on && !state_out) ? reinterpret_cast<uint32_t*>(sc.P[l]) : (uint32_t*)nullptr);
        else ATT_DISPATCH_SH(attn_fwd, (size_t)4 * NH * L * sizeof(float), sc.QKV[l], row_env, row_t, offsets, R, L, sc.P[l], sc.ATT[l], dc, l, sc.PM[l]);
        if (state_out && l == nl - 1) {
            static_assert(tD == 32, "prefix_last_rows_kernel maps 32 columns to 32 threads");
            float *ATTc = sc.T0, *Hc = sc.T1;
            int32_t *env_c = reinterpret_cast<int32_t*>(sc.T2), *t_c = env_c + B;
            hipLaunchKernelGGL(prefix_last_rows_kernel, dim3(cdiv(B, 8)), dim3(256), 0, s, (const float*)sc.ATT[l], (const float*)sc.H[l], row_env, row_t, offsets,
                               lens, B, ATTc, Hc, env_c, t_c);
            LayerFwdArgs fa{ATTc, Hc, y, nullptr, nullptr, sc.XH1[l], sc.RS1[l], sc.H1N[l], sc.FF1[l], sc.XH2[l], sc.RS2[l], sc.H[l + 1], nullptr,
                            env_c, t_c, B, l};
            if (dc.on) CIRS_LAUNCH_SPREAD(layer_rows_fwd<true>, cdiv(B, 32), 40 * 1024, 0, s, fa, dc);
            else CIRS_LAUNCH_SPREAD(layer_rows_fwd<false>, cdiv(B, 32), 40 * 1024, 0, s, fa, dc);
            continue;
        }
        LayerFwdArgs fa{sc.ATT[l], sc.H[l], y, l + 1 < nl ? w->layer[l + 1].in_proj_w : nullptr, l + 1 < nl ? w->layer[l + 1].in_proj_b : nullptr,
                        sc.XH1[l], sc.RS1[l], sc.H1N[l], sc.FF1[l], sc.XH2[l], sc.RS2[l], sc.H[l + 1], l + 1 < nl ? sc.QKV[l + 1] : nullptr,
                        row_env, row_t, R, l};
        if (dc.on) CIRS_LAUNCH_SPREAD(layer_rows_fwd<true>, cdiv(R, 32), 40 * 1024, 0, s, fa, dc);
        else CIRS_LAUNCH_SPREAD(layer_rows_fwd<false>, cdiv(R, 32), 40 * 1024, 0, s, fa, dc);
    }
    CIRS_CHECK_LAUNCH("tracker forward recompute");
    if (state_out) {
        hipLaunchKernelGGL(prefix_decoder_kernel, dim3(cdiv(B, 4)), dim3(256), 0, s, (const float*)sc.H[nl], lens, B, S, w->dec_w, w->dec_b,
                           state_out, (long)state_stride);
        CIRS_CHECK_LAUNCH("prefix_decoder_kernel");
        return CIRS_OK;
    }
    float* dH = sc.T0;
    if (top_last) {
        hipLaunchKernelGGL(dstate_last_rows, g1((long)B * S), dim3(256), 0, s, dstate_last, lens, B, S, sc.G);
        launch_rows_gemm(false, sc.G, S, w->dec_w, tD, nullptr, B, S, tD, 0, nullptr, 0, dH, tD, s);
    } else {
        if (dstate_last) hipLaunchKernelGGL(dstate_last_full, g1((long)R * S), dim3(256), 0, s, dstate_last, row_env, offsets, lens, R, S, sc.G);
        else hipLaunchKernelGGL(gather_dstate, g1((long)R * S), dim3(256), 0, s, dstate, row_env, row_t, R, S, B, sc.G);
        launch_rows_gemm_dw(dwl, sc.H[nl], tD, S, tD, grads->dec_w, grads->dec_b, sc.partial, false, sc.G, S, w->dec_w, tD, nullptr, R, S, tD, 0, nullptr, 0,
                            dH, tD, s);
    }
    for (int l = nl - 1; l >= 0; --l) {
        const cirs_tracker_layer& y = w->layer[l];
        const cirs_tracker_layer_grads& gy = grads->layer[l];
        if (top_last && l == nl - 1) {
            float* dB1 = dc.on ? sc.T4 : dY1c;
            LayerBwdArgs ba{sc.T0, nullptr, nullptr, nullptr, sc.T0, 0, y, sc.XH2[l], sc.RS2[l], sc.FF1[l], sc.XH1[l], sc.RS1[l], sc.T3, sc.dFF1, sc.T1, dY1c, dB1,
                            sc.T5, env_c, t_c, B, l};
            if (dc.on) CIRS_LAUNCH_SPREAD(layer_rows_bwd<true>, cdiv(B, 32), 40 * 1024, 0, s, ba, dc);
            else CIRS_LAUNCH_SPREAD(layer_rows_bwd<false>, cdiv(B, 32), 40 * 1024, 0, s, ba, dc);
            DwBatch bt{};
            dw_batch_add(bt, dwl, sc.G, S, sc.H[nl], tD, R, S, tD, grads->dec_w, grads->dec_b, 0, sc.partial);
            dw_batch_add(bt, dwl, sc.T0, tD, sc.XH2[l], tD, R, tD, tD, gy.norm2_w, gy.norm2_b, 1, sc.partial);
            dw_batch_add(bt, dwl, sc.T3, tD, sc.FF1[l], tH, R, tD, tH, gy.lin2_w, gy.lin2_b, 0, sc.partial);
            dw_batch_add(bt, dwl, sc.dFF1, tH, sc.H1N[l], tD, R, tH, tD, gy.lin1_w, gy.lin1_b, 0, sc.partial);
            dw_batch_add(bt, dwl, sc.T1, tD, sc.XH1[l], tD, R, tD, tD, gy.norm1_w, gy.norm1_b, 1, sc.partial);
            dw_batch_add(bt, dwl, dB1, tD, sc.ATT[l], tD, R, tD, tD, gy.out_proj_w, gy.out_proj_b, 0, sc.partial);
            dw_batch_launch(bt, R, s, B);
            ATT_LAST(attn_last_bwd, (const float*)sc.QKV[l], (const float*)sc.T5, (const float*)dY1c, (const float*)att_stats, offsets, lens, B, L, sc.dQKV,
                     sc.T2, dc, l);
            continue;
        }
        const bool pre = l + 1 < nl;
        float* dB1 = dc.on ? sc.T4 : sc.T2;
        LayerBwdArgs ba{sc.T0, pre ? sc.T2 : nullptr, pre ? sc.dQKV : nullptr, pre ? w->layer[l + 1].in_proj_w : nullptr, sc.T0, 0, y,
                        sc.XH2[l], sc.RS2[l], sc.FF1[l], sc.XH1[l], sc.RS1[l], sc.T3, sc.dFF1, sc.T1, sc.T2, dB1, sc.T5, row_env, row_t, R, l};
        if (dc.on) CIRS_LAUNCH_SPREAD(layer_rows_bwd<true>, cdiv(R, 32), 40 * 1024, 0, s, ba, dc);
        else CIRS_LAUNCH_SPREAD(layer_rows_bwd<false>, cdiv(R, 32), 40 * 1024, 0, s, ba, dc);
        DwBatch bt{};
        if (pre) dw_batch_add(bt, dwl, sc.dQKV, 96, sc.H[l + 1], tD, R, 96, tD, grads->layer[l + 1].in_proj_w, grads->layer[l + 1].in_proj_b, 0, sc.partial);
        dw_batch_add(bt, dwl, sc.T0, tD, sc.XH2[l], tD, R, tD, tD, gy.norm2_w, gy.norm2_b, 1, sc.partial);
        dw_batch_add(bt, dwl, sc.T3, tD, sc.FF1[l], tH, R, tD, tH, gy.lin2_w, gy.lin2_b, 0, sc.partial);
        dw_batch_add(bt, dwl, sc.dFF1, tH, sc.H1N[l], tD, R, tH, tD, gy.lin1_w, gy.lin1_b, 0, sc.partial);
        dw_batch_add(bt, dwl, sc.T1, tD, sc.XH1[l], tD, R, tD, tD, gy.norm1_w, gy.norm1_b, 1, sc.partial);
        dw_batch_add(bt, dwl, dB1, tD, sc.ATT[l], tD, R, tD, tD, gy.out_proj_w, gy.out_proj_b, 0, sc.partial);
        dw_batch_launch(bt, R, s);
        const float* dATT = sc.T5;
        if (ep) {
            ATT_EP(attn_bwd_ep, true, (const float*)sc.QKV[l], dATT, offsets, lens, L, sc.dQKV, dc, l, dc.on ? reinterpret_cast<const uint32_t*>(sc.P[l]) : (const uint32_t*)nullptr);
        } else {
            ATT_DISPATCH_SH(attn_bwd_q, (size_t)4 * NH * L * sizeof(float), sc.QKV[l], sc.P[l], dATT, row_env, row_t, offsets, R, L, sc.dS, sc.dQKV,
                            (const float*)sc.PM[l], dc.inv);
            ATT_DISPATCH(attn_bwd_kv, sc.QKV[l], dc.on ? sc.PM[l] : sc.P[l], sc.dS, dATT, row_env, row_t, offsets, lens, R, L, sc.dQKV);
        }
    }
    {
        LayerBwdArgs ba{};
        ba.dY1p = sc.T2; ba.dQKVp = sc.dQKV; ba.winp = w->layer[0].in_proj_w; ba.dHout = sc.T0; ba.only_pre = 1;
        ba.row_env = row_env; ba.row_t = row_t; ba.R = R;
        if (dc.on) CIRS_LAUNCH_SPREAD(layer_rows_bwd<true>, cdiv(R, 32), 40 * 1024, 0, s, ba, dc);
        else CIRS_LAUNCH_SPREAD(layer_rows_bwd<false>, cdiv(R, 32), 40 * 1024, 0, s, ba, dc);
    }
    CIRS_CHECK_LAUNCH("tracker backward layers");
    float* DU = sc.T1;
    float* EU = sc.H[nl];
    float* DPRE = sc.H1N[0];
    float* CU = sc.QKV[0];
    float* CI = sc.QKV[0] + (size_t)R * tD;
    int32_t* key_user = (int32_t*)sc.RS1[0];
    int32_t* key_item = (int32_t*)sc.RS2[0];
    const bool merged = B <= R;
    const int slot_rpw = R >= (1 << 17) ? 8 : 1;
    hipLaunchKernelGGL(slot_bwd, dim3(cdiv(R, 4 * slot_rpw)), dim3(256), 0, s, *w, dH, users, act, rew, row_env, row_t, R, B, DU, EU, DPRE,
                       sc.GIN, CU, CI, key_user, key_item, merged ? CI + (size_t)R * tD : nullptr, slot_rpw, 5.656854249492381f);
    if (merged) {
        if (int rc = emb_scatter_merged(key_item, users, lens, CI, R, B, cfg->n_items, cfg->n_users, grads->emb_item, grads->emb_user, sc.sort,
                                        emb_sort_bytes(R + B), s)) return rc;
    } else {
        int32_t* keys_c = (int32_t*)sc.T0;
        float* contrib_c = sc.T2;
        CIRS_HIP(hipMemsetAsync(keys_c, 0xFF, sizeof(int32_t) * (size_t)B, s));
        hipLaunchKernelGGL(compact_user_rows, dim3(cdiv(R, 8)), dim3(256), 0, s, row_env, row_t, users, (const float*)CU, R, keys_c, contrib_c);
        if (int rc = emb_scatter_sorted(keys_c, contrib_c, B, cfg->n_users, grads->emb_user, sc.sort, emb_sort_bytes(R), s)) return rc;
        if (int rc = emb_scatter_sorted(key_item, CI, R, cfg->n_items, grads->emb_item, sc.sort, emb_sort_bytes(R), s)) return rc;
    }
    DwBatch bt{};
    dw_batch_add(bt, dwl, sc.dQKV, 96, sc.H[0], tD, R, 96, tD, grads->layer[0].in_proj_w, grads->layer[0].in_proj_b, 0, sc.partial);
    dw_batch_add(bt, dwl, DU, tD, EU, tD, R, tD, tD, grads->ffn_user_w, grads->ffn_user_b, 0, sc.partial);
    dw_batch_add(bt, dwl, DPRE, tD, sc.GIN, tD + 1, R, tD, tD + 1, grads->gate_w, grads->gate_b, 0, sc.partial);
    dw_batch_launch(bt, R, s);
    launch_dw_list_final(dwl, R, sc.partial, s);
    CIRS_CHECK_LAUNCH("tracker backward slots");
#undef ATT_LAST
#undef ATT_LAST1
#undef ATT_DISPATCH
#undef ATT_EP
#undef ATT_EP1
#undef ATT_DISPATCH_SH
    return CIRS_OK;
}

extern "C" int cirs_tracker_backward(const cirs_tracker_cfg* cfg, const cirs_tracker_weights* w, const cirs_tracker_state* st,
                                     const int32_t* users, const int64_t* act, const double* rew, const int32_t* row_env,
                                     const int32_t* row_t, const int32_t* offsets, const int32_t* lens, int32_t n_rows,
                                     const float* dstate, const cirs_tracker_grads* grads, void* workspace,
                                     int64_t workspace_bytes, void* stream) {
    CIRS_REQUIRE(users && act && rew && dstate && grads, "null argument");
    return tracker_rows_impl(cfg, w, st, users, act, rew, row_env, row_t, offsets, lens, n_rows, dstate, grads, workspace, workspace_bytes, stream,
                             nullptr, 0);
}

extern "C" int cirs_tracker_backward_last(const cirs_tracker_cfg* cfg, const cirs_tracker_weights* w, const cirs_tracker_state* st,
                                          const int32_t* users, const int64_t* act, const double* rew, const int32_t* row_env,
                                          const int32_t* row_t, const int32_t* offsets, const int32_t* lens, int32_t n_rows,
                                          const float* dstate_last, const cirs_tracker_grads* grads, void* workspace,
                                          int64_t workspace_bytes, void* stream) {
    CIRS_REQUIRE(users && act && rew && dstate_last && grads, "null argument");
    return tracker_rows_impl(cfg, w, st, users, act, rew, row_env, row_t, offsets, lens, n_rows, nullptr, grads, workspace, workspace_bytes, stream,
                             nullptr, 0, dstate_last);
}

extern "C" int cirs_tracker_prefix_states(const cirs_tracker_cfg* cfg, const cirs_tracker_weights* w, const cirs_tracker_state* st,
                                          const int32_t* row_env, const int32_t* row_t, const int32_t* offsets, const int32_t* lens,
                                          int32_t n_rows, float* state_out, int64_t state_stride, void* workspace, int64_t workspace_bytes,
                                          void* stream) {
    CIRS_REQUIRE(state_out && state_stride >= (cfg ? cfg->dim_state : 0), "bad state_out");
    return tracker_rows_impl(cfg, w, st, nullptr, nullptr, nullptr, row_env, row_t, offsets, lens, n_rows, nullptr, nullptr, workspace, workspace_bytes,
                             stream, state_out, state_stride);
}

int cirs::tracker_prefix_states_trunk(const cirs_tracker_cfg* cfg, const cirs_tracker_weights* w, const cirs_tracker_state* st, const int32_t* row_env,
                                      const int32_t* row_t, const int32_t* offsets, const int32_t* lens, int32_t n_rows, float* state_out, int64_t state_stride,
                                      void* workspace, int64_t workspace_bytes, void* stream, const TrunkFuse* tf, int* fused) {
    CIRS_REQUIRE(state_out && state_stride >= (cfg ? cfg->dim_state : 0) && fused, "bad state_out");
    *fused = 0;
    return tracker_rows_impl(cfg, w, st, nullptr, nullptr, nullptr, row_env, row_t, offsets, lens, n_rows, nullptr, nullptr, workspace, workspace_bytes,
                             stream, state_out, state_stride, nullptr, tf, fused);
}

extern "C" int64_t cirs_embedding_scatter_workspace_bytes(int64_t n_rows) { return (int64_t)cirs::emb_sort_bytes(n_rows) + 1024; }

extern "C" int cirs_embedding_scatter(const int32_t* keys, const float* contrib, int64_t n_rows, int32_t n_table_rows, float* grad_table,
                                      void* workspace, int64_t workspace_bytes, void* stream) {
    using namespace cirs;
    CIRS_REQUIRE(keys && contrib && grad_table && workspace && n_rows > 0 && n_table_rows > 0, "bad arguments");
    CIRS_REQUIRE(n_rows < (1ll << 31), "too many rows");
    CIRS_REQUIRE(workspace_bytes >= cirs_embedding_scatter_workspace_bytes(n_rows), "workspace too small");
    void* ws = (void*)(((uintptr_t)workspace + 255) & ~(uintptr_t)255);
    return emb_scatter_sorted(keys, contrib, (int)n_rows, n_table_rows, grad_table, ws, (size_t)workspace_bytes - 256, (hipStream_t)stream);
}
```

### cirs-codes_amd/csrc/tracker_rows.h

```cpp
#pragma once
#include <hipcub/hipcub.hpp>
#include "small_gemm.h"
#include "internal.h"

namespace cirs {
typedef float f32x4 __attribute__((ext_vector_type(4)));

constexpr int tD = 32, tH = 128;

constexpr int kMaxDwBatch = 8;
struct DwBatchJob { const float* dY; int ldy; const float* X; int ldx; int O, K, tile_begin; float* partial; };
struct DwBatch { DwBatchJob j[kMaxDwBatch]; int n, total_tiles; };
static __global__ __launch_bounds__(64) void dw_batch_kernel(DwBatch jobs, int R, int rows_per_slab) {
    int ji = 0;
    for (; ji + 1 < jobs.n && (int)blockIdx.x >= jobs.j[ji + 1].tile_begin; ++ji) {}
    const DwBatchJob& jb = jobs.j[ji];
    dw_gemm_body((int)blockIdx.x - jb.tile_begin, blockIdx.y, jb.dY, jb.ldy, jb.X, jb.ldx, R, jb.O, jb.K, rows_per_slab, jb.partial);
}
static inline void dw_batch_add(DwBatch& b, DwList& list, const float* dY, int ldy, const float* X, int ldx, int R, int O, int K, float* dW,
                                float* db, int diag, float* partial) {
    const int slabs = dwg_slabs(R);
    DwListJob& lj = list.j[list.n++];
    lj.O = O; lj.K = K; lj.part_off = list.part_floats; lj.diag = diag; lj.dW = dW; lj.db = db;
    DwBatchJob& jb = b.j[b.n++];
    jb.dY = dY; jb.ldy = ldy; jb.X = X; jb.ldx = ldx; jb.O = O; jb.K = K; jb.tile_begin = b.total_tiles; jb.partial = partial + lj.part_off;
    b.total_tiles += cdiv(O, 32) * cdiv(K, 32);
    list.part_floats += slabs * O * (K + 1);
    list.total_out += O * (K + 1);
}
static inline void dw_batch_launch(const DwBatch& b, int R, hipStream_t s, int R_rows = -1) {
    if (!b.n) return;
    if (R_rows < 0) R_rows = R;
    const int slabs = dwg_slabs(R);
    int rows_per_slab = (R_rows + slabs - 1) / slabs;
    rows_per_slab = (rows_per_slab + 15) & ~15;
    hipLaunchKernelGGL(dw_batch_kernel, dim3(b.total_tiles, slabs), dim3(64), 0, s, b, R_rows, rows_per_slab);
}

static __global__ __launch_bounds__(256) void gather_dstate(const float* __restrict__ dstate, const int32_t* __restrict__ row_env,
                                                     const int32_t* __restrict__ row_t, int R, int S, int B, float* __restrict__ G) {
    const long i = blockIdx.x * (long)blockDim.x + threadIdx.x;
    if (i >= (long)R * S) return;
    const int r = (int)(i / S), s = (int)(i % S);
    G[i] = dstate[((size_t)row_t[r] * B + row_env[r]) * S + s];
}

__device__ __forceinline__ float lane_bcast(float x, int k) {
    return __builtin_bit_cast(float, __builtin_amdgcn_readlane(__builtin_bit_cast(int, x), k));
}

static __global__ __launch_bounds__(256) void slot_bwd(cirs_tracker_weights w, const float* __restrict__ dH0, const int32_t* __restrict__ users,
                                                const int64_t* __restrict__ act, const double* __restrict__ rew,
                                                const int32_t* __restrict__ row_env, const int32_t* __restrict__ row_t, int R, int B,
                                                float* __restrict__ DU, float* __restrict__ EU, float* __restrict__ DPRE,
                                                float* __restrict__ GIN, float* __restrict__ CU, float* __restrict__ CI,
                                                int32_t* __restrict__ key_user, int32_t* __restrict__ key_item,
                                                float* __restrict__ contrib_c ,
                                                int rows_per_wave, float in_scale ) {
    const int lane = threadIdx.x & 63;
    __shared__ float sG[tD * (tD + 1)];
    for (int q = threadIdx.x; q < tD * (tD + 1); q += 256) sG[q] = w.gate_w[q];
    __syncthreads();
    for (int it_r = 0; it_r < rows_per_wave; ++it_r) {
    const int r = (blockIdx.x * rows_per_wave + it_r) * 4 + (threadIdx.x >> 6);
    if (r >= R) return;
    const int b = row_env[r], p = row_t[r];
    const int d = lane & 31;
    const float dx = dH0[(size_t)r * tD + d] * in_scale;
    if (p == 0) {
        const int u = users[b];
        const float eu = w.emb_user[(size_t)u * tD + d];
        if (lane < tD) {
            DU[(size_t)r * tD + d] = dx; EU[(size_t)r * tD + d] = eu;
            DPRE[(size_t)r * tD + d] = 0.f;
        }
        if (lane <= tD) GIN[(size_t)r * (tD + 1) + lane] = 0.f;
        float acc = 0.f;
#pragma unroll
        for (int o = 0; o < tD; ++o) acc = __builtin_fmaf(lane_bcast(dx, o), w.ffn_user_w[(size_t)o * tD + d], acc);
        if (lane < tD) {
            CU[(size_t)r * tD + d] = acc; CI[(size_t)r * tD + d] = 0.f;
            if (contrib_c) contrib_c[(size_t)b * tD + d] = acc;
        }
        if (lane == 0) { key_user[r] = u; key_item[r] = -1; }
    } else {
        const size_t ti = (size_t)(p - 1) * B + b;
        const long it = act[ti];
        const float rw = (float)rew[ti];
        const float a = w.emb_item[(size_t)it * tD + d];
        const float* gw = sG + d * (tD + 1);
        float pre = w.gate_b[d];
        pre = __builtin_fmaf(gw[0], rw, pre);
#pragma unroll
        for (int k = 0; k < tD; ++k) pre = __builtin_fmaf(gw[1 + k], lane_bcast(a, k), pre);
        const float g = 1.0f / (1.0f + expf(-pre));
        const float dpre = dx * a * g * (1.0f - g);
        if (lane < tD) {
            DPRE[(size_t)r * tD + d] = dpre;
            DU[(size_t)r * tD + d] = 0.f; EU[(size_t)r * tD + d] = 0.f;
            GIN[(size_t)r * (tD + 1) + 1 + d] = a;
        }
        if (lane == 0) GIN[(size_t)r * (tD + 1)] = rw;
        float acc = dx * g;
#pragma unroll
        for (int o = 0; o < tD; ++o) acc = __builtin_fmaf(lane_bcast(dpre, o), sG[o * (tD + 1) + 1 + d], acc);
        if (lane < tD) { CI[(size_t)r * tD + d] = acc; CU[(size_t)r * tD + d] = 0.f; }
        if (lane == 0) { key_item[r] = (int32_t)it; key_user[r] = -1; }
    }
    }
}

static __global__ __launch_bounds__(256) void scatter_keys_kernel(const int32_t* __restrict__ keys, int R, int n_table,
                                                           uint32_t* __restrict__ keys_u, int32_t* __restrict__ rows) {
    const int r = blockIdx.x * blockDim.x + threadIdx.x;
    if (r >= R) return;
    const int32_t k = keys[r];
    keys_u[r] = (k < 0 || k >= n_table) ? (uint32_t)n_table : (uint32_t)k;
    rows[r] = r;
}

static __global__ __launch_bounds__(256) void compact_user_rows(const int32_t* __restrict__ row_env, const int32_t* __restrict__ row_t,
                                                         const int32_t* __restrict__ users, const float* __restrict__ CU, int R,
                                                         int32_t* __restrict__ keys_c, float* __restrict__ contrib_c) {
    const int d = threadIdx.x & 31;
    const int r = blockIdx.x * 8 + (threadIdx.x >> 5);
    if (r >= R || row_t[r] != 0) return;
    const int b = row_env[r];
    contrib_c[(size_t)b * tD + d] = CU[(size_t)r * tD + d];
    if (d == 0) keys_c[b] = users[b];
}

constexpr int kSubRun = 64;
static __global__ __launch_bounds__(256) void emb_subrun_kernel(const uint32_t* __restrict__ ks, const int32_t* __restrict__ rs,
                                                         const float* __restrict__ contrib, int R, int n_table, float* __restrict__ part) {
    const int d = threadIdx.x & 31, half = (threadIdx.x >> 5) & 1;
    const int p = blockIdx.x * 8 + (threadIdx.x >> 5);
    const bool in = p < R;
    const uint32_t key = in ? ks[p] : 0xffffffffu;
    const bool start = in && key < (uint32_t)n_table && ((p % kSubRun) == 0 || ks[p - 1] != key);
    const int end = min(R, (p / kSubRun + 1) * kSubRun);
    const int q0 = p + d, q1 = p + 32 + d;
    const bool s0 = start && q0 < end && ks[q0] == key, s1 = start && q1 < end && ks[q1] == key;
    const int r0 = s0 ? rs[q0] : 0, r1 = s1 ? rs[q1] : 0;
    const unsigned long long m0 = __ballot(s0), m1 = __ballot(s1);
    if (!start) return;
    const uint32_t h0 = (uint32_t)(m0 >> (32 * half)), h1 = (uint32_t)(m1 >> (32 * half));
    const int n = h0 == 0xffffffffu ? 32 + (h1 == 0xffffffffu ? 32 : __builtin_ctz(~h1)) : __builtin_ctz(~h0);
    float acc = 0.f;
    for (int q = 0; q < n; q += 16) {
        float t[16];
#pragma unroll
        for (int u = 0; u < 16; ++u) {
            const int qq = q + u;
            const int row = __shfl(qq < 32 ? r0 : r1, (qq & 31) + 32 * half, CIRS_WAVE);
            t[u] = qq < n ? contrib[(size_t)row * tD + d] : 0.f;
        }
#pragma unroll
        for (int u = 0; u < 16; ++u) acc += (q + u < n) ? t[u] : 0.f;
    }
    part[(size_t)p * tD + d] = acc;
}

static __global__ __launch_bounds__(256) void emb_segment_sum_kernel(const uint32_t* __restrict__ ks, const float* __restrict__ part, int R,
                                                              int n_table, float* __restrict__ g_emb, int n_first = 0x7fffffff,
                                                              float* __restrict__ g_second = nullptr) {
    const int d = threadIdx.x & 31;
    const int p = blockIdx.x * 8 + (threadIdx.x >> 5);
    if (p >= R) return;
    const uint32_t key = ks[p];
    if (key >= (uint32_t)n_table || (p > 0 && ks[p - 1] == key)) return;
    float acc = part[(size_t)p * tD + d];
    for (int q = (p / kSubRun + 1) * kSubRun; q < R; q += 8 * kSubRun) {
        float t8[8];
        int n_ok = 0;
#pragma unroll
        for (int u = 0; u < 8; ++u) {
            const int qq = q + u * kSubRun;
            const bool ok = (n_ok == u) && qq < R && ks[qq] == key;
            t8[u] = ok ? part[(size_t)qq * tD + d] : 0.f;
            n_ok += ok;
        }
#pragma unroll
        for (int u = 0; u < 8; ++u) acc += (u < n_ok) ? t8[u] : 0.f;
        if (n_ok < 8) break;
    }
    if (key < (uint32_t)n_first) g_emb[(size_t)key * tD + d] = acc;
    else g_second[(size_t)(key - (uint32_t)n_first) * tD + d] = acc;
}

static size_t emb_sort_bytes(long R) { return (size_t)R * (64 + 4 * tD) + (1u << 20); }

static int emb_scatter_sorted(const int32_t* keys, const float* contrib, int R, int n_table, float* g_emb, void* scratch,
                              size_t scratch_bytes, hipStream_t s) {
    static_assert(tD == 32, "emb_segment_sum_kernel maps one lane per embedding dimension");
    uint32_t* k_in = (uint32_t*)scratch;
    uint32_t* k_out = k_in + R;
    int32_t* r_in = (int32_t*)(k_out + R);
    int32_t* r_out = r_in + R;
    float* part = (float*)(((uintptr_t)(r_out + R) + 255) & ~(uintptr_t)255);
    char* temp = (char*)(((uintptr_t)(part + (size_t)R * tD) + 255) & ~(uintptr_t)255);
    const size_t avail = scratch_bytes - (size_t)(temp - (char*)scratch);
    int end_bit = 1;
    while ((1u << end_bit) <= (uint32_t)n_table && end_bit < 32) ++end_bit;
    size_t need = 0;
    CIRS_HIP(hipcub::DeviceRadixSort::SortPairs(nullptr, need, k_in, k_out, r_in, r_out, R, 0, end_bit, s));
    CIRS_REQUIRE(need <= avail, "embedding scatter: sort scratch too small");
    CIRS_HIP(hipMemsetAsync(g_emb, 0, (size_t)n_table * tD * sizeof(float), s));
    hipLaunchKernelGGL(scatter_keys_kernel, dim3(cdiv(R, 256)), dim3(256), 0, s, keys, R, n_table, k_in, r_in);
    CIRS_HIP(hipcub::DeviceRadixSort::SortPairs(temp, need, k_in, k_out, r_in, r_out, R, 0, end_bit, s));
    hipLaunchKernelGGL(emb_subrun_kernel, dim3(cdiv(R, 8)), dim3(256), 0, s, k_out, r_out, contrib, R, n_table, part);
    hipLaunchKernelGGL(emb_segment_sum_kernel, dim3(cdiv(R, 8)), dim3(256), 0, s, k_out, (const float*)part, R, n_table, g_emb);
    CIRS_CHECK_LAUNCH("emb_segment_sum_kernel");
    return CIRS_OK;
}

static __global__ __launch_bounds__(256) void scatter_keys2_kernel(const int32_t* __restrict__ key_item, const int32_t* __restrict__ users,
                                                            const int32_t* __restrict__ lens, int R, int B, int n_items, int n_users,
                                                            uint32_t* __restrict__ keys_u, int32_t* __restrict__ rows,
                                                            float* __restrict__ zero_table , long zero_floats) {
    const int p = blockIdx.x * blockDim.x + threadIdx.x;
    if (zero_table)
        for (long i = (long)p * 4; i < zero_floats; i += (long)gridDim.x * blockDim.x * 4) *reinterpret_cast<f32x4*>(zero_table + i) = f32x4{0.f, 0.f, 0.f, 0.f};
    if (p >= R + B) return;
    const uint32_t sent = (uint32_t)n_items + (uint32_t)n_users;
    uint32_t k = sent;
    if (p < R) {
        const int32_t v = key_item[p];
        if (v >= 0 && v < n_items) k = (uint32_t)v;
    } else {
        const int b = p - R;
        const int32_t u = users[b];
        if (lens[b] > 0 && u >= 0 && u < n_users) k = (uint32_t)n_items + (uint32_t)u;
    }
    keys_u[p] = k;
    rows[p] = p;
}
static int emb_scatter_merged(const int32_t* key_item, const int32_t* users, const int32_t* lens, const float* contrib, int R, int B,
                              int n_items, int n_users, float* g_item, float* g_user, void* scratch, size_t scratch_bytes, hipStream_t s) {
    const int N = R + B, n_table = n_items + n_users;
    uint32_t* k_in = (uint32_t*)scratch;
    uint32_t* k_out = k_in + N;
    int32_t* r_in = (int32_t*)(k_out + N);
    int32_t* r_out = r_in + N;
    float* part = (float*)(((uintptr_t)(r_out + N) + 255) & ~(uintptr_t)255);
    char* temp = (char*)(((uintptr_t)(part + (size_t)N * tD) + 255) & ~(uintptr_t)255);
    const size_t avail = scratch_bytes - (size_t)(temp - (char*)scratch);
    int end_bit = 1;
    while ((1u << end_bit) <= (uint32_t)n_table && end_bit < 32) ++end_bit;
    size_t need = 0;
    CIRS_HIP(hipcub::DeviceRadixSort::SortPairs(nullptr, need, k_in, k_out, r_in, r_out, N, 0, end_bit, s));
    CIRS_REQUIRE(need <= avail, "embedding scatter: sort scratch too small");
    float* zero_table = nullptr;
    if (g_user + (size_t)n_users * tD == g_item) zero_table = g_user;
    else if (g_item + (size_t)n_items * tD == g_user) zero_table = g_item;
    if (zero_table && ((uintptr_t)zero_table & 15)) zero_table = nullptr;
    if (!zero_table) {
        CIRS_HIP(hipMemsetAsync(g_item, 0, (size_t)n_items * tD * sizeof(float), s));
        CIRS_HIP(hipMemsetAsync(g_user, 0, (size_t)n_users * tD * sizeof(float), s));
    }
    hipLaunchKernelGGL(scatter_keys2_kernel, dim3(cdiv(N, 256)), dim3(256), 0, s, key_item, users, lens, R, B, n_items, n_users, k_in, r_in, zero_table,
                       (long)n_table * tD);
    CIRS_HIP(hipcub::DeviceRadixSort::SortPairs(temp, need, k_in, k_out, r_in, r_out, N, 0, end_bit, s));
    hipLaunchKernelGGL(emb_subrun_kernel, dim3(cdiv(N, 8)), dim3(256), 0, s, k_out, r_out, contrib, N, n_table, part);
    hipLaunchKernelGGL(emb_segment_sum_kernel, dim3(cdiv(N, 8)), dim3(256), 0, s, k_out, (const float*)part, N, n_table, g_item, n_items, g_user);
    CIRS_CHECK_LAUNCH("emb_segment_sum_kernel (merged)");
    return CIRS_OK;
}

}
```

Baseline: 6.006 million.

## Co-schedule weight-grad GEMM waves with attention backward and add custom radix sort

Fuses the per-layer batched weight-gradient GEMM into the attention-backward kernel. Each block gets extra waves that work through dW tiles while wave 0 runs the per-sequence attention backward. dQKV is double-buffered across layers so the in_proj dW of layer l+1 can read its dQKV while layer l writes the other buffer. It also replaces hipcub radix sort in the embedding scatter with a custom two-pass 8-bit radix sort that zeroes the gradient table in the same kernel when the table is small. An environment variable can force the old serial paths. The change trades extra scratch memory and higher per-block register and LDS pressure for fewer launches and overlap of the two workloads.

Result: no change. 6.049 million, median of 6 (+0.7%).

```diff
diff --git a/cirs-codes_amd/csrc/small_gemm.h b/cirs-codes_amd/csrc/small_gemm.h
--- a/cirs-codes_amd/csrc/small_gemm.h
+++ b/cirs-codes_amd/csrc/small_gemm.h
@@ -104,7 +104,7 @@
 
 __device__ __forceinline__ void dw_gemm_body(int bx, int slab, const float* __restrict__ dY, int ldy, const float* __restrict__ X, int ldx, int R,
                                              int O, int K, int rows_per_slab, float* __restrict__ partial) {
-    const int lane = threadIdx.x, hi = lane >> 5, lo = lane & 31;
+    const int lane = threadIdx.x & 63, hi = lane >> 5, lo = lane & 31;
     const int k_tiles = (K + 31) / 32;
     const int o0 = (bx / k_tiles) * 32, k0 = (bx % k_tiles) * 32;
     const int r_beg = slab * rows_per_slab, r_end = min(R, r_beg + rows_per_slab);
diff --git a/cirs-codes_amd/csrc/tracker_bwd.hip b/cirs-codes_amd/csrc/tracker_bwd.hip
--- a/cirs-codes_amd/csrc/tracker_bwd.hip
+++ b/cirs-codes_amd/csrc/tracker_bwd.hip
@@ -426,15 +426,15 @@
     }
 }
 
-template <int NH, bool kDrop>
-__global__ __launch_bounds__(64) void attn_bwd_ep(const float* __restrict__ QKV, const float* __restrict__ dATT,
-                                                  const int32_t* __restrict__ offsets, const int32_t* __restrict__ lens, int Lp,
-                                                  float* __restrict__ dQKV, DropCfg dc, int layer,
-                                                  const uint32_t* __restrict__ keep_in ) {
+template <int NH, bool kDrop, bool kOwnWave>
+__device__ __forceinline__ void attn_bwd_ep_body(int b , const float* __restrict__ QKV, const float* __restrict__ dATT,
+                                                 const int32_t* __restrict__ offsets, const int32_t* __restrict__ lens, int Lp,
+                                                 float* __restrict__ dQKV, const DropCfg& dc, int layer,
+                                                 const uint32_t* __restrict__ keep_in ) {
     using G = EpGeo<NH>;
     constexpr int HPL = G::HPL, DPL = G::DPL, HD = G::HD, SL = G::SL;
     extern __shared__ __attribute__((aligned(16))) float smem[];
-    const int b = blockIdx.x, len = lens[b];
+    const int len = lens[b];
     if (len <= 0) return;
     const int lane = threadIdx.x, hg = lane / SL, slot = lane - hg * SL;
     const int base = offsets[b], STR = G::strip(Lp);
@@ -464,7 +464,7 @@
         ep_stage(sQKV + 32 * 96, QKV + (size_t)(base + 32) * 96, len - 32, 96, 96, lane, 64);
         ep_stage(sdA + 32 * tD, dATT + (size_t)(base + 32) * tD, len - 32, tD, tD, lane, 64);
     }
-    __syncthreads();
+    if (kOwnWave) ep_wave_sync(); else __syncthreads();
     CIRS_BSTAMP(40);
     const float scale = 1.0f / sqrtf((float)HD), qs = scale * 1.4426950408889634f;
     const float dinv = kDrop ? dc.inv : 1.0f;
@@ -576,7 +576,7 @@
         if (actA) ep_store(dQKV + (size_t)(base + pA) * 96 + hg * DPL, dqA, scale);
         if (actB) ep_store(dQKV + (size_t)(base + pB) * 96 + hg * DPL, dqB, scale);
     }
-    __syncthreads();
+    if (kOwnWave) ep_wave_sync(); else __syncthreads();
     CIRS_BSTAMP(41);
     for (int s0 = 0; 2 * s0 < len; s0 += SL) {
         const int jA = s0 + slot, jB = len - 1 - jA;
@@ -632,6 +632,26 @@
     }
     CIRS_BSTAMP(42);
     CIRS_BWG(layer == 1, 1);
+}
+template <int NH, bool kDrop>
+__global__ __launch_bounds__(64) void attn_bwd_ep(const float* __restrict__ QKV, const float* __restrict__ dATT,
+                                                  const int32_t* __restrict__ offsets, const int32_t* __restrict__ lens, int Lp,
+                                                  float* __restrict__ dQKV, DropCfg dc, int layer, const uint32_t* __restrict__ keep_in) {
+    attn_bwd_ep_body<NH, kDrop, false>(blockIdx.x, QKV, dATT, offsets, lens, Lp, dQKV, dc, layer, keep_in);
+}
+constexpr int kDwWaves = 1;
+template <int NH, bool kDrop>
+__global__ __launch_bounds__(64 * (1 + kDwWaves)) void attn_bwd_ep_dw(const float* __restrict__ QKV, const float* __restrict__ dATT,
+                                                      const int32_t* __restrict__ offsets, const int32_t* __restrict__ lens, int Lp,
+                                                      float* __restrict__ dQKV, DropCfg dc, int layer, const uint32_t* __restrict__ keep_in,
+                                                      DwBatch jobs, int n_items, int R, int rows_per_slab) {
+    if (threadIdx.x < 64) {
+        attn_bwd_ep_body<NH, kDrop, true>(blockIdx.x, QKV, dATT, offsets, lens, Lp, dQKV, dc, layer, keep_in);
+        return;
+    }
+    const int nw = (int)gridDim.x * kDwWaves;
+    for (int q = (int)blockIdx.x + (int)gridDim.x * ((int)(threadIdx.x >> 6) - 1); q < n_items; q += nw)
+        dw_batch_body(jobs, q % jobs.total_tiles, q / jobs.total_tiles, R, rows_per_slab);
 }
 #undef EP_KEEP
 
@@ -1038,6 +1058,8 @@
     float* LC;
     float* PM[CIRS_MAX_TRACKER_LAYERS];
     void* sort;
+    float* dQKVb;
+    float* dqkv(int layer) const { return (layer & 1) ? dQKVb : dQKV; }
 };
 
 constexpr int kLastFloats = tD + 16 + 2 + 2;
@@ -1061,6 +1083,7 @@
     f += (size_t)R * (tD + 1);
     f += (size_t)R * kLastFloats;
     f += emb_sort_bytes(R + cfg->n_env) / 4 + 64;
+    f += (size_t)R * 96;
     return f + 64 * 32;
 }
 
@@ -1084,6 +1107,7 @@
     s.GIN = take((size_t)R * (tD + 1));
     s.LC = take((size_t)R * kLastFloats);
     s.sort = (void*)take(emb_sort_bytes(R + cfg->n_env) / 4 + 64);
+    s.dQKVb = take((size_t)R * 96);
     return s;
 }
 
@@ -1667,12 +1691,13 @@
 template <typename K> static inline void lds_optin(K k, size_t dyn) {
     if (dyn > 8 * 1024) (void)hipFuncSetAttribute(reinterpret_cast<const void*>(k), hipFuncAttributeMaxDynamicSharedMemorySize, (int)dyn);
 }
-#define CIRS_LAUNCH_SPREAD(KERNEL, GRID, STATIC_B, DYN_B, STREAM, ...)                                  \
+#define CIRS_LAUNCH_SPREAD_T(KERNEL, GRID, THREADS, STATIC_B, DYN_B, STREAM, ...)                        \
     do {                                                                                               \
         const size_t dyn_ = spread_dyn_lds((long)(GRID), (STATIC_B), (DYN_B));                         \
         if (dyn_ != (size_t)(DYN_B)) lds_optin(KERNEL, dyn_);                                          \
-        hipLaunchKernelGGL(KERNEL, dim3(GRID), dim3(64), dyn_, STREAM, __VA_ARGS__);                   \
+        hipLaunchKernelGGL(KERNEL, dim3(GRID), dim3(THREADS), dyn_, STREAM, __VA_ARGS__);              \
     } while (0)
+#define CIRS_LAUNCH_SPREAD(KERNEL, GRID, STATIC_B, DYN_B, STREAM, ...) CIRS_LAUNCH_SPREAD_T(KERNEL, GRID, 64, STATIC_B, DYN_B, STREAM, __VA_ARGS__)
 
 static int tracker_rows_impl(const cirs_tracker_cfg* cfg, const cirs_tracker_weights* w, const cirs_tracker_state* st,
                              const int32_t* users, const int64_t* act, const double* rew, const int32_t* row_env,
@@ -1693,6 +1718,7 @@
     BwdScratch sc = carve_bwd(workspace, cfg, n_carve);
     auto g1 = [&](long n) { return dim3(cdiv(n, 256)); };
 
+    const int serial = state_out ? 0 : tracker_bwd_serial();
     DwList dwl{};
 #define ATT_DISPATCH_SH(KERNEL, SHMEM, ...)                                                               \
     do {                                                                                                  \
@@ -1713,20 +1739,21 @@
         }
     };
     const bool ep = L <= 64 && ep_bytes(true) <= 64 * 1024 && !getenv("CIRS_TRACKER_ATTN_ROWS");
-#define ATT_EP1(KERNEL, N, BWD, ...)                                                                                            \
+#define ATT_EP1(KERNEL, N, BWD, THREADS, ...)                                                                                   \
     do {                                                                                                                        \
-        if (dc.on) CIRS_LAUNCH_SPREAD((KERNEL<N, true>), B, 0, ep_bytes(BWD), s, __VA_ARGS__);       \
-        else CIRS_LAUNCH_SPREAD((KERNEL<N, false>), B, 0, ep_bytes(BWD), s, __VA_ARGS__);           \
+        if (dc.on) CIRS_LAUNCH_SPREAD_T((KERNEL<N, true>), B, THREADS, 0, ep_bytes(BWD), s, __VA_ARGS__);       \
+        else CIRS_LAUNCH_SPREAD_T((KERNEL<N, false>), B, THREADS, 0, ep_bytes(BWD), s, __VA_ARGS__);           \
     } while (0)
-#define ATT_EP(KERNEL, BWD, ...)                                  \
-    do {                                                          \
-        switch (NH) {                                             \
-            case 1: ATT_EP1(KERNEL, 1, BWD, __VA_ARGS__); break;  \
-            case 2: ATT_EP1(KERNEL, 2, BWD, __VA_ARGS__); break;  \
-            case 4: ATT_EP1(KERNEL, 4, BWD, __VA_ARGS__); break;  \
-            default: ATT_EP1(KERNEL, 8, BWD, __VA_ARGS__); break; \
-        }                                                         \
+#define ATT_EP_T(KERNEL, BWD, THREADS, ...)                                  \
+    do {                                                                     \
+        switch (NH) {                                                        \
+            case 1: ATT_EP1(KERNEL, 1, BWD, THREADS, __VA_ARGS__); break;    \
+            case 2: ATT_EP1(KERNEL, 2, BWD, THREADS, __VA_ARGS__); break;    \
+            case 4: ATT_EP1(KERNEL, 4, BWD, THREADS, __VA_ARGS__); break;    \
+            default: ATT_EP1(KERNEL, 8, BWD, THREADS, __VA_ARGS__); break;   \
+        }                                                                    \
     } while (0)
+#define ATT_EP(KERNEL, BWD, ...) ATT_EP_T(KERNEL, BWD, 64, __VA_ARGS__)
 
     DropCfg dc{};
     if (cfg->dropout_p > 0.f) {
@@ -1847,36 +1874,43 @@
             dw_batch_add(bt, dwl, sc.T1, tD, sc.XH1[l], tD, R, tD, tD, gy.norm1_w, gy.norm1_b, 1, sc.partial);
             dw_batch_add(bt, dwl, dB1, tD, sc.ATT[l], tD, R, tD, tD, gy.out_proj_w, gy.out_proj_b, 0, sc.partial);
             dw_batch_launch(bt, R, s, B);
-            ATT_LAST(attn_last_bwd, (const float*)sc.QKV[l], (const float*)sc.T5, (const float*)dY1c, (const float*)att_stats, offsets, lens, B, L, sc.dQKV,
+            ATT_LAST(attn_last_bwd, (const float*)sc.QKV[l], (const float*)sc.T5, (const float*)dY1c, (const float*)att_stats, offsets, lens, B, L, sc.dqkv(l),
                      sc.T2, dc, l);
             continue;
         }
         const bool pre = l + 1 < nl;
         float* dB1 = dc.on ? sc.T4 : sc.T2;
-        LayerBwdArgs ba{sc.T0, pre ? sc.T2 : nullptr, pre ? sc.dQKV : nullptr, pre ? w->layer[l + 1].in_proj_w : nullptr, sc.T0, 0, y,
+        float *dQKV_up = sc.dqkv(l + 1), *dQKV_l = sc.dqkv(l);
+        LayerBwdArgs ba{sc.T0, pre ? sc.T2 : nullptr, pre ? dQKV_up : nullptr, pre ? w->layer[l + 1].in_proj_w : nullptr, sc.T0, 0, y,
                         sc.XH2[l], sc.RS2[l], sc.FF1[l], sc.XH1[l], sc.RS1[l], sc.T3, sc.dFF1, sc.T1, sc.T2, dB1, sc.T5, row_env, row_t, R, l};
         if (dc.on) CIRS_LAUNCH_SPREAD(layer_rows_bwd<true>, cdiv(R, 32), 40 * 1024, 0, s, ba, dc);
         else CIRS_LAUNCH_SPREAD(layer_rows_bwd<false>, cdiv(R, 32), 40 * 1024, 0, s, ba, dc);
         DwBatch bt{};
-        if (pre) dw_batch_add(bt, dwl, sc.dQKV, 96, sc.H[l + 1], tD, R, 96, tD, grads->layer[l + 1].in_proj_w, grads->layer[l + 1].in_proj_b, 0, sc.partial);
+        if (pre) dw_batch_add(bt, dwl, dQKV_up, 96, sc.H[l + 1], tD, R, 96, tD, grads->layer[l + 1].in_proj_w, grads->layer[l + 1].in_proj_b, 0, sc.partial);
         dw_batch_add(bt, dwl, sc.T0, tD, sc.XH2[l], tD, R, tD, tD, gy.norm2_w, gy.norm2_b, 1, sc.partial);
         dw_batch_add(bt, dwl, sc.T3, tD, sc.FF1[l], tH, R, tD, tH, gy.lin2_w, gy.lin2_b, 0, sc.partial);
         dw_batch_add(bt, dwl, sc.dFF1, tH, sc.H1N[l], tD, R, tH, tD, gy.lin1_w, gy.lin1_b, 0, sc.partial);
         dw_batch_add(bt, dwl, sc.T1, tD, sc.XH1[l], tD, R, tD, tD, gy.norm1_w, gy.norm1_b, 1, sc.partial);
         dw_batch_add(bt, dwl, dB1, tD, sc.ATT[l], tD, R, tD, tD, gy.out_proj_w, gy.out_proj_b, 0, sc.partial);
+        const float* dATT = sc.T5;
+        const uint32_t* keep = dc.on ? reinterpret_cast<const uint32_t*>(sc.P[l]) : (const uint32_t*)nullptr;
+        if (ep && !(serial & kSerialAttn) && dw_batch_rows_per_slab(R, R) <= 256) {
+            ATT_EP_T(attn_bwd_ep_dw, true, 64 * (1 + kDwWaves), (const float*)sc.QKV[l], dATT, offsets, lens, L, dQKV_l, dc, l, keep, bt, bt.total_tiles * dwg_slabs(R), R,
+                     dw_batch_rows_per_slab(R, R));
+            continue;
+        }
         dw_batch_launch(bt, R, s);
-        const float* dATT = sc.T5;
         if (ep) {
-            ATT_EP(attn_bwd_ep, true, (const float*)sc.QKV[l], dATT, offsets, lens, L, sc.dQKV, dc, l, dc.on ? reinterpret_cast<const uint32_t*>(sc.P[l]) : (const uint32_t*)nullptr);
+            ATT_EP(attn_bwd_ep, true, (const float*)sc.QKV[l], dATT, offsets, lens, L, dQKV_l, dc, l, keep);
         } else {
-            ATT_DISPATCH_SH(attn_bwd_q, (size_t)4 * NH * L * sizeof(float), sc.QKV[l], sc.P[l], dATT, row_env, row_t, offsets, R, L, sc.dS, sc.dQKV,
+            ATT_DISPATCH_SH(attn_bwd_q, (size_t)4 * NH * L * sizeof(float), sc.QKV[l], sc.P[l], dATT, row_env, row_t, offsets, R, L, sc.dS, dQKV_l,
                             (const float*)sc.PM[l], dc.inv);
-            ATT_DISPATCH(attn_bwd_kv, sc.QKV[l], dc.on ? sc.PM[l] : sc.P[l], sc.dS, dATT, row_env, row_t, offsets, lens, R, L, sc.dQKV);
+            ATT_DISPATCH(attn_bwd_kv, sc.QKV[l], dc.on ? sc.PM[l] : sc.P[l], sc.dS, dATT, row_env, row_t, offsets, lens, R, L, dQKV_l);
         }
     }
     {
         LayerBwdArgs ba{};
-        ba.dY1p = sc.T2; ba.dQKVp = sc.dQKV; ba.winp = w->layer[0].in_proj_w; ba.dHout = sc.T0; ba.only_pre = 1;
+        ba.dY1p = sc.T2; ba.dQKVp = sc.dqkv(0); ba.winp = w->layer[0].in_proj_w; ba.dHout = sc.T0; ba.only_pre = 1;
         ba.row_env = row_env; ba.row_t = row_t; ba.R = R;
         if (dc.on) CIRS_LAUNCH_SPREAD(layer_rows_bwd<true>, cdiv(R, 32), 40 * 1024, 0, s, ba, dc);
         else CIRS_LAUNCH_SPREAD(layer_rows_bwd<false>, cdiv(R, 32), 40 * 1024, 0, s, ba, dc);
@@ -1895,17 +1929,17 @@
                        sc.GIN, CU, CI, key_user, key_item, merged ? CI + (size_t)R * tD : nullptr, slot_rpw, 5.656854249492381f);
     if (merged) {
         if (int rc = emb_scatter_merged(key_item, users, lens, CI, R, B, cfg->n_items, cfg->n_users, grads->emb_item, grads->emb_user, sc.sort,
-                                        emb_sort_bytes(R + B), s)) return rc;
+                                        emb_sort_bytes(R + B), s, serial)) return rc;
     } else {
         int32_t* keys_c = (int32_t*)sc.T0;
         float* contrib_c = sc.T2;
         CIRS_HIP(hipMemsetAsync(keys_c, 0xFF, sizeof(int32_t) * (size_t)B, s));
         hipLaunchKernelGGL(compact_user_rows, dim3(cdiv(R, 8)), dim3(256), 0, s, row_env, row_t, users, (const float*)CU, R, keys_c, contrib_c);
-        if (int rc = emb_scatter_sorted(keys_c, contrib_c, B, cfg->n_users, grads->emb_user, sc.sort, emb_sort_bytes(R), s)) return rc;
-        if (int rc = emb_scatter_sorted(key_item, CI, R, cfg->n_items, grads->emb_item, sc.sort, emb_sort_bytes(R), s)) return rc;
+        if (int rc = emb_scatter_sorted(keys_c, contrib_c, B, cfg->n_users, grads->emb_user, sc.sort, emb_sort_bytes(R), s, serial)) return rc;
+        if (int rc = emb_scatter_sorted(key_item, CI, R, cfg->n_items, grads->emb_item, sc.sort, emb_sort_bytes(R), s, serial)) return rc;
     }
     DwBatch bt{};
-    dw_batch_add(bt, dwl, sc.dQKV, 96, sc.H[0], tD, R, 96, tD, grads->layer[0].in_proj_w, grads->layer[0].in_proj_b, 0, sc.partial);
+    dw_batch_add(bt, dwl, sc.dqkv(0), 96, sc.H[0], tD, R, 96, tD, grads->layer[0].in_proj_w, grads->layer[0].in_proj_b, 0, sc.partial);
     dw_batch_add(bt, dwl, DU, tD, EU, tD, R, tD, tD, grads->ffn_user_w, grads->ffn_user_b, 0, sc.partial);
     dw_batch_add(bt, dwl, DPRE, tD, sc.GIN, tD + 1, R, tD, tD + 1, grads->gate_w, grads->gate_b, 0, sc.partial);
     dw_batch_launch(bt, R, s);
@@ -1915,6 +1949,7 @@
 #undef ATT_LAST1
 #undef ATT_DISPATCH
 #undef ATT_EP
+#undef ATT_EP_T
 #undef ATT_EP1
 #undef ATT_DISPATCH_SH
     return CIRS_OK;
@@ -1967,5 +2002,5 @@
     CIRS_REQUIRE(n_rows < (1ll << 31), "too many rows");
     CIRS_REQUIRE(workspace_bytes >= cirs_embedding_scatter_workspace_bytes(n_rows), "workspace too small");
     void* ws = (void*)(((uintptr_t)workspace + 255) & ~(uintptr_t)255);
-    return emb_scatter_sorted(keys, contrib, (int)n_rows, n_table_rows, grad_table, ws, (size_t)workspace_bytes - 256, (hipStream_t)stream);
-}
+    return emb_scatter_sorted(keys, contrib, (int)n_rows, n_table_rows, grad_table, ws, (size_t)workspace_bytes - 256, (hipStream_t)stream, tracker_bwd_serial());
+}
diff --git a/cirs-codes_amd/csrc/tracker_rows.h b/cirs-codes_amd/csrc/tracker_rows.h
--- a/cirs-codes_amd/csrc/tracker_rows.h
+++ b/cirs-codes_amd/csrc/tracker_rows.h
@@ -11,11 +11,18 @@
 constexpr int kMaxDwBatch = 8;
 struct DwBatchJob { const float* dY; int ldy; const float* X; int ldx; int O, K, tile_begin; float* partial; };
 struct DwBatch { DwBatchJob j[kMaxDwBatch]; int n, total_tiles; };
+__device__ __forceinline__ void dw_batch_body(const DwBatch& jobs, int tile, int slab, int R, int rows_per_slab) {
+    int ji = 0;
+    for (; ji + 1 < jobs.n && tile >= jobs.j[ji + 1].tile_begin; ++ji) {}
+    const DwBatchJob& jb = jobs.j[ji];
+    dw_gemm_body(tile - jb.tile_begin, slab, jb.dY, jb.ldy, jb.X, jb.ldx, R, jb.O, jb.K, rows_per_slab, jb.partial);
+}
 static __global__ __launch_bounds__(64) void dw_batch_kernel(DwBatch jobs, int R, int rows_per_slab) {
-    int ji = 0;
-    for (; ji + 1 < jobs.n && (int)blockIdx.x >= jobs.j[ji + 1].tile_begin; ++ji) {}
-    const DwBatchJob& jb = jobs.j[ji];
-    dw_gemm_body((int)blockIdx.x - jb.tile_begin, blockIdx.y, jb.dY, jb.ldy, jb.X, jb.ldx, R, jb.O, jb.K, rows_per_slab, jb.partial);
+    dw_batch_body(jobs, blockIdx.x, blockIdx.y, R, rows_per_slab);
+}
+static inline int dw_batch_rows_per_slab(int R, int R_rows) {
+    const int slabs = dwg_slabs(R);
+    return ((R_rows + slabs - 1) / slabs + 15) & ~15;
 }
 static inline void dw_batch_add(DwBatch& b, DwList& list, const float* dY, int ldy, const float* X, int ldx, int R, int O, int K, float* dW,
                                 float* db, int diag, float* partial) {
@@ -31,10 +38,7 @@
 static inline void dw_batch_launch(const DwBatch& b, int R, hipStream_t s, int R_rows = -1) {
     if (!b.n) return;
     if (R_rows < 0) R_rows = R;
-    const int slabs = dwg_slabs(R);
-    int rows_per_slab = (R_rows + slabs - 1) / slabs;
-    rows_per_slab = (rows_per_slab + 15) & ~15;
-    hipLaunchKernelGGL(dw_batch_kernel, dim3(b.total_tiles, slabs), dim3(64), 0, s, b, R_rows, rows_per_slab);
+    hipLaunchKernelGGL(dw_batch_kernel, dim3(b.total_tiles, dwg_slabs(R)), dim3(64), 0, s, b, R_rows, dw_batch_rows_per_slab(R, R_rows));
 }
 
 static __global__ __launch_bounds__(256) void gather_dstate(const float* __restrict__ dstate, const int32_t* __restrict__ row_env,
@@ -188,10 +192,155 @@
     else g_second[(size_t)(key - (uint32_t)n_first) * tD + d] = acc;
 }
 
+constexpr int kRdxBlock = 1024;
+constexpr int kRdxMaxBlocks = 128;
+struct EmbKeySrc { const int32_t *key_item, *users, *lens; int R, B, n_items, n_users; };
+__device__ __forceinline__ uint32_t emb_key_at(const EmbKeySrc& ks, int p) {
+    uint32_t k = (uint32_t)ks.n_items + (uint32_t)ks.n_users;
+    if (p < ks.R) {
+        const int32_t v = ks.key_item[p];
+        if (v >= 0 && v < ks.n_items) k = (uint32_t)v;
+    } else {
+        const int b = p - ks.R;
+        const int32_t u = ks.users[b];
+        if (ks.lens[b] > 0 && u >= 0 && u < ks.n_users) k = (uint32_t)ks.n_items + (uint32_t)u;
+    }
+    return k;
+}
+static __global__ __launch_bounds__(256) void emb_rdx_keys_kernel(EmbKeySrc ks, int nb, uint32_t* __restrict__ keys_u, int* __restrict__ hist0,
+                                                           int* __restrict__ hist1, float* __restrict__ zero_table , long zero_floats) {
+    __shared__ int sh[256];
+    const int tid = threadIdx.x, blk = blockIdx.x;
+    if (zero_table)
+        for (long i = ((long)blk * 256 + tid) * 4; i < zero_floats; i += (long)gridDim.x * 256 * 4) *reinterpret_cast<f32x4*>(zero_table + i) = f32x4{0.f, 0.f, 0.f, 0.f};
+    if (blk >= nb) return;
+    sh[tid] = 0;
+    hist1[blk * 256 + tid] = 0;
+    __syncthreads();
+    const int N = ks.R + ks.B;
+#pragma unroll
+    for (int j = 0; j < kRdxBlock / 256; ++j) {
+        const int p = blk * kRdxBlock + j * 256 + tid;
+        if (p < N) {
+            const uint32_t k = emb_key_at(ks, p);
+            keys_u[p] = k;
+            atomicAdd(&sh[k & 255u], 1);
+        }
+    }
+    __syncthreads();
+    hist0[blk * 256 + tid] = sh[tid];
+}
+template <bool kFirst>
+static __global__ __launch_bounds__(256) void emb_rdx_scatter(const uint32_t* __restrict__ k_src, const int32_t* __restrict__ r_src ,
+                                                       int N, int nb, const int* __restrict__ hist ,
+                                                       int* __restrict__ hist_next ,
+                                                       uint32_t* __restrict__ k_dst, int32_t* __restrict__ r_dst) {
+    typedef hipcub::BlockScan<int, 256> Scan;
+    __shared__ typename Scan::TempStorage scan_tmp;
+    __shared__ int wcnt[4][256];
+    const int tid = threadIdx.x, w = tid >> 6, lane = tid & 63, blk = blockIdx.x;
+    constexpr int shift = kFirst ? 0 : 8;
+    int total = 0, before = 0;
+    for (int b0 = 0; b0 < nb; b0 += 8) {
+        int c[8];
+#pragma unroll
+        for (int u = 0; u < 8; ++u) c[u] = b0 + u < nb ? hist[(b0 + u) * 256 + tid] : 0;
+#pragma unroll
+        for (int u = 0; u < 8; ++u) {
+            total += c[u];
+            before += b0 + u < blk ? c[u] : 0;
+        }
+    }
+    int smaller;
+    Scan(scan_tmp).ExclusiveSum(total, smaller);
+    const int gbase = smaller + before;
+#pragma unroll
+    for (int q = 0; q < 4; ++q) wcnt[q][tid] = 0;
+    __syncthreads();
+    uint32_t key[4];
+    int row[4], rank[4];
+    unsigned long long same[4];
+#pragma unroll
+    for (int j = 0; j < 4; ++j) {
+        const int p = blk * kRdxBlock + w * 256 + j * 64 + lane;
+        const bool act = p < N;
+        key[j] = act ? k_src[p] : 0u;
+        row[j] = kFirst ? p : (act ? r_src[p] : 0);
+        const uint32_t d = (key[j] >> shift) & 255u;
+        unsigned long long m = __ballot(act);
+#pragma unroll
+        for (int bit = 0; bit < 8; ++bit) {
+            const bool one = (d >> bit) & 1u;
+            const unsigned long long bb = __ballot(one);
+            m &= one ? bb : ~bb;
+        }
+        if (kFirst) {
+            unsigned long long m2 = m;
+#pragma unroll
+            for (int bit = 8; bit < 16; ++bit) {
+                const bool one = (key[j] >> bit) & 1u;
+                const unsigned long long bb = __ballot(one);
+                m2 &= one ? bb : ~bb;
+            }
+            same[j] = m2;
+        }
+        const int below = __popcll(m & ((1ull << lane) - 1ull));
+        const int seen = act ? wcnt[w][d] : 0;
+        __builtin_amdgcn_wave_barrier();
+        if (act && below == 0) wcnt[w][d] = seen + __popcll(m);
+        __builtin_amdgcn_wave_barrier();
+        rank[j] = seen + below;
+    }
+    __syncthreads();
+    {
+        int run = gbase;
+#pragma unroll
+        for (int q = 0; q < 4; ++q) { const int c = wcnt[q][tid]; wcnt[q][tid] = run; run += c; }
+    }
+    __syncthreads();
+#pragma unroll
+    for (int j = 0; j < 4; ++j) {
+        const int p = blk * kRdxBlock + w * 256 + j * 64 + lane;
+        const int dest = wcnt[w][(key[j] >> shift) & 255u] + rank[j];
+        const bool ok = p < N && (unsigned)dest < (unsigned)N;
+        if (ok) {
+            k_dst[dest] = key[j];
+            r_dst[dest] = row[j];
+        }
+        if (kFirst) {
+            const bool odd = (dest / kRdxBlock) & 1;
+            const unsigned long long bo = __ballot(odd), g = same[j] & (odd ? bo : ~bo) & __ballot(ok);
+            if (ok && (g & ((1ull << lane) - 1ull)) == 0) atomicAdd(&hist_next[(dest / kRdxBlock) * 256 + (int)((key[j] >> 8) & 255u)], __popcll(g));
+        }
+    }
+}
+constexpr int kSerialAttn = 1, kSerialSort = 2;
+static inline int tracker_bwd_serial() {
+    const char* e = getenv("CIRS_TRACKER_BWD_SERIAL");
+    if (!e || !e[0] || (e[0] == '0' && !e[1])) return 0;
+    if (e[0] == 'a' && !e[1]) return kSerialAttn;
+    if (e[0] == 'c' && !e[1]) return kSerialSort;
+    return kSerialAttn | kSerialSort;
+}
+static inline bool emb_rdx_order(const EmbKeySrc& ks, int serial, uint32_t* k_a, int32_t* r_a, uint32_t* k_b, int32_t* r_b, char* temp, size_t avail,
+                                 float* zero_table, long zero_floats, hipStream_t s) {
+    const long N = (long)ks.R + ks.B, n_table = (long)ks.n_items + ks.n_users;
+    const int nb = (int)cdiv(N, (long)kRdxBlock);
+    if (serial < 0) serial = tracker_bwd_serial();
+    if ((serial & kSerialSort) || n_table >= 65536 || nb > kRdxMaxBlocks || avail < (size_t)2 * nb * 256 * sizeof(int)) return false;
+    int* hist0 = reinterpret_cast<int*>(temp);
+    int* hist1 = hist0 + (size_t)nb * 256;
+    const int clear_blocks = zero_table ? (int)std::min<long>(cdiv(zero_floats, 256L * 4 * 4), 1024) : 0;
+    hipLaunchKernelGGL(emb_rdx_keys_kernel, dim3(std::max(nb, clear_blocks)), dim3(256), 0, s, ks, nb, k_a, hist0, hist1, zero_table, zero_floats);
+    hipLaunchKernelGGL(emb_rdx_scatter<true>, dim3(nb), dim3(256), 0, s, (const uint32_t*)k_a, (const int32_t*)nullptr, (int)N, nb, (const int*)hist0, hist1, k_b, r_b);
+    hipLaunchKernelGGL(emb_rdx_scatter<false>, dim3(nb), dim3(256), 0, s, (const uint32_t*)k_b, (const int32_t*)r_b, (int)N, nb, (const int*)hist1, (int*)nullptr, k_a, r_a);
+    return true;
+}
+
 static size_t emb_sort_bytes(long R) { return (size_t)R * (64 + 4 * tD) + (1u << 20); }
 
 static int emb_scatter_sorted(const int32_t* keys, const float* contrib, int R, int n_table, float* g_emb, void* scratch,
-                              size_t scratch_bytes, hipStream_t s) {
+                              size_t scratch_bytes, hipStream_t s, int serial = -1 ) {
     static_assert(tD == 32, "emb_segment_sum_kernel maps one lane per embedding dimension");
     uint32_t* k_in = (uint32_t*)scratch;
     uint32_t* k_out = k_in + R;
@@ -200,14 +349,21 @@
     float* part = (float*)(((uintptr_t)(r_out + R) + 255) & ~(uintptr_t)255);
     char* temp = (char*)(((uintptr_t)(part + (size_t)R * tD) + 255) & ~(uintptr_t)255);
     const size_t avail = scratch_bytes - (size_t)(temp - (char*)scratch);
-    int end_bit = 1;
-    while ((1u << end_bit) <= (uint32_t)n_table && end_bit < 32) ++end_bit;
-    size_t need = 0;
-    CIRS_HIP(hipcub::DeviceRadixSort::SortPairs(nullptr, need, k_in, k_out, r_in, r_out, R, 0, end_bit, s));
-    CIRS_REQUIRE(need <= avail, "embedding scatter: sort scratch too small");
-    CIRS_HIP(hipMemsetAsync(g_emb, 0, (size_t)n_table * tD * sizeof(float), s));
-    hipLaunchKernelGGL(scatter_keys_kernel, dim3(cdiv(R, 256)), dim3(256), 0, s, keys, R, n_table, k_in, r_in);
-    CIRS_HIP(hipcub::DeviceRadixSort::SortPairs(temp, need, k_in, k_out, r_in, r_out, R, 0, end_bit, s));
+    float* zero_table = ((uintptr_t)g_emb & 15) ? nullptr : g_emb;
+    const EmbKeySrc ks{keys, nullptr, nullptr, R, 0, n_table, 0};
+    if (!zero_table) CIRS_HIP(hipMemsetAsync(g_emb, 0, (size_t)n_table * tD * sizeof(float), s));
+    if (emb_rdx_order(ks, serial, k_in, r_in, k_out, r_out, temp, avail, zero_table, (long)n_table * tD, s)) {
+        k_out = k_in; r_out = r_in;
+    } else {
+        int end_bit = 1;
+        while ((1u << end_bit) <= (uint32_t)n_table && end_bit < 32) ++end_bit;
+        size_t need = 0;
+        CIRS_HIP(hipcub::DeviceRadixSort::SortPairs(nullptr, need, k_in, k_out, r_in, r_out, R, 0, end_bit, s));
+        CIRS_REQUIRE(need <= avail, "embedding scatter: sort scratch too small");
+        if (zero_table) CIRS_HIP(hipMemsetAsync(g_emb, 0, (size_t)n_table * tD * sizeof(float), s));
+        hipLaunchKernelGGL(scatter_keys_kernel, dim3(cdiv(R, 256)), dim3(256), 0, s, keys, R, n_table, k_in, r_in);
+        CIRS_HIP(hipcub::DeviceRadixSort::SortPairs(temp, need, k_in, k_out, r_in, r_out, R, 0, end_bit, s));
+    }
     hipLaunchKernelGGL(emb_subrun_kernel, dim3(cdiv(R, 8)), dim3(256), 0, s, k_out, r_out, contrib, R, n_table, part);
     hipLaunchKernelGGL(emb_segment_sum_kernel, dim3(cdiv(R, 8)), dim3(256), 0, s, k_out, (const float*)part, R, n_table, g_emb);
     CIRS_CHECK_LAUNCH("emb_segment_sum_kernel");
@@ -236,7 +392,8 @@
     rows[p] = p;
 }
 static int emb_scatter_merged(const int32_t* key_item, const int32_t* users, const int32_t* lens, const float* contrib, int R, int B,
-                              int n_items, int n_users, float* g_item, float* g_user, void* scratch, size_t scratch_bytes, hipStream_t s) {
+                              int n_items, int n_users, float* g_item, float* g_user, void* scratch, size_t scratch_bytes, hipStream_t s,
+                              int serial = -1 ) {
     const int N = R + B, n_table = n_items + n_users;
     uint32_t* k_in = (uint32_t*)scratch;
     uint32_t* k_out = k_in + N;
@@ -245,11 +402,6 @@
     float* part = (float*)(((uintptr_t)(r_out + N) + 255) & ~(uintptr_t)255);
     char* temp = (char*)(((uintptr_t)(part + (size_t)N * tD) + 255) & ~(uintptr_t)255);
     const size_t avail = scratch_bytes - (size_t)(temp - (char*)scratch);
-    int end_bit = 1;
-    while ((1u << end_bit) <= (uint32_t)n_table && end_bit < 32) ++end_bit;
-    size_t need = 0;
-    CIRS_HIP(hipcub::DeviceRadixSort::SortPairs(nullptr, need, k_in, k_out, r_in, r_out, N, 0, end_bit, s));
-    CIRS_REQUIRE(need <= avail, "embedding scatter: sort scratch too small");
     float* zero_table = nullptr;
     if (g_user + (size_t)n_users * tD == g_item) zero_table = g_user;
     else if (g_item + (size_t)n_items * tD == g_user) zero_table = g_item;
@@ -258,9 +410,19 @@
         CIRS_HIP(hipMemsetAsync(g_item, 0, (size_t)n_items * tD * sizeof(float), s));
         CIRS_HIP(hipMemsetAsync(g_user, 0, (size_t)n_users * tD * sizeof(float), s));
     }
-    hipLaunchKernelGGL(scatter_keys2_kernel, dim3(cdiv(N, 256)), dim3(256), 0, s, key_item, users, lens, R, B, n_items, n_users, k_in, r_in, zero_table,
-                       (long)n_table * tD);
-    CIRS_HIP(hipcub::DeviceRadixSort::SortPairs(temp, need, k_in, k_out, r_in, r_out, N, 0, end_bit, s));
+    const EmbKeySrc ks{key_item, users, lens, R, B, n_items, n_users};
+    if (emb_rdx_order(ks, serial, k_in, r_in, k_out, r_out, temp, avail, zero_table, (long)n_table * tD, s)) {
+        k_out = k_in; r_out = r_in;
+    } else {
+        int end_bit = 1;
+        while ((1u << end_bit) <= (uint32_t)n_table && end_bit < 32) ++end_bit;
+        size_t need = 0;
+        CIRS_HIP(hipcub::DeviceRadixSort::SortPairs(nullptr, need, k_in, k_out, r_in, r_out, N, 0, end_bit, s));
+        CIRS_REQUIRE(need <= avail, "embedding scatter: sort scratch too small");
+        hipLaunchKernelGGL(scatter_keys2_kernel, dim3(cdiv(N, 256)), dim3(256), 0, s, key_item, users, lens, R, B, n_items, n_users, k_in, r_in, zero_table,
+                           (long)n_table * tD);
+        CIRS_HIP(hipcub::DeviceRadixSort::SortPairs(temp, need, k_in, k_out, r_in, r_out, N, 0, end_bit, s));
+    }
     hipLaunchKernelGGL(emb_subrun_kernel, dim3(cdiv(N, 8)), dim3(256), 0, s, k_out, r_out, contrib, N, n_table, part);
     hipLaunchKernelGGL(emb_segment_sum_kernel, dim3(cdiv(N, 8)), dim3(256), 0, s, k_out, (const float*)part, N, n_table, g_item, n_items, g_user);
     CIRS_CHECK_LAUNCH("emb_segment_sum_kernel (merged)");
```
